# SamsungLabs/nb-asr

Measured on AMD Instinct MI355X. Metric: utterances_per_sec, higher is better.
Workload: dtype f32

## Files before the change

### nb_asr_amd/csrc/gemm_conv_split.hip

```cpp
#include "storage.h"

#include <cstdlib>

#include <type_traits>

namespace nbasr {

typedef float floatx4 __attribute__((ext_vector_type(4)));

constexpr int PB_CI = 16, PB_TAPS = 8;
constexpr int pb_frames(int nj) { return 64 * nj; }
constexpr int pb_rows(int mi) { return 32 * mi; }
constexpr int PB_THREADS = 512;

struct SplitBf16x3 {
    static constexpr int NS = 3;
    typedef __bf16 vec8 __attribute__((ext_vector_type(8)));
    static constexpr bool SCALED = false;
    __host__ __device__ static constexpr int taps_per_step(int stride) { return stride == 1 ? 4 : 2; }
    __device__ static __forceinline__ void split(float v, unsigned short (&s)[NS]) {
        const __bf16 hi = static_cast<__bf16>(v);
        const float r1 = v - static_cast<float>(hi);
        const __bf16 mid = static_cast<__bf16>(r1);
        const __bf16 lo = static_cast<__bf16>(r1 - static_cast<float>(mid));
        s[0] = __builtin_bit_cast(unsigned short, hi);
        s[1] = __builtin_bit_cast(unsigned short, mid);
        s[2] = __builtin_bit_cast(unsigned short, lo);
    }
    __device__ static __forceinline__ floatx4 mfma(vec8 a, vec8 b, floatx4 c) {
        return __builtin_amdgcn_mfma_f32_16x16x32_bf16(a, b, c, 0, 0, 0);
    }
    static constexpr const char* NAME = "nbasr_dense_conv1d_packed(bf16x3)";
};

struct SplitF16x2 {
    static constexpr int NS = 2;
    typedef _Float16 vec8 __attribute__((ext_vector_type(8)));
    static constexpr bool SCALED = true;
    __host__ __device__ static constexpr int taps_per_step(int) { return 4; }
    __device__ static __forceinline__ void split(float v, unsigned short (&s)[NS]) {
        const _Float16 hi = static_cast<_Float16>(v);
        const _Float16 lo = static_cast<_Float16>(v - static_cast<float>(hi));
        s[0] = __builtin_bit_cast(unsigned short, hi);
        s[1] = __builtin_bit_cast(unsigned short, lo);
    }
    __device__ static __forceinline__ floatx4 mfma(vec8 a, vec8 b, floatx4 c) {
        return __builtin_amdgcn_mfma_f32_16x16x32_f16(a, b, c, 0, 0, 0);
    }
    static constexpr const char* NAME = "nbasr_dense_conv1d_packed(f16x2)";
};

struct PlainBf16 {
    static constexpr int NS = 1;
    typedef __bf16 vec8 __attribute__((ext_vector_type(8)));
    static constexpr bool SCALED = false;
    __host__ __device__ static constexpr int taps_per_step(int) { return 8; }
    __device__ static __forceinline__ void split(float v, unsigned short (&s)[NS]) {
        s[0] = __builtin_bit_cast(unsigned short, static_cast<__bf16>(v));
    }
    __device__ static __forceinline__ floatx4 mfma(vec8 a, vec8 b, floatx4 c) {
        return __builtin_amdgcn_mfma_f32_16x16x32_bf16(a, b, c, 0, 0, 0);
    }
    static constexpr const char* NAME = "nbasr_dense_conv1d_packed(bf16)";
};

template <class P> constexpr bool has_image_path() { return P::SCALED || P::NS == 1; }

template <class P> constexpr size_t pb_group_bytes(int mi) { return static_cast<size_t>(P::NS) * PB_TAPS * pb_rows(mi) * PB_CI * 2; }

template <class P, int S, int MI = 4, int NJ = 4>
struct GeoP {
    static constexpr int PBM = pb_rows(MI);
    static constexpr int PBN = pb_frames(NJ);
    static constexpr int TP = P::taps_per_step(S);
    static constexpr int QSTEPS = PB_TAPS / TP;
    static constexpr int A_STEP_BYTES = P::NS * TP * PBM * PB_CI * 2;
    static constexpr int XR = (PBN - 1) * S + PB_TAPS;
    static constexpr int XRH = (XR + 1) / 2;
    static constexpr int ROWS = (S == 1) ? XR : 2 * XRH;
    static constexpr int RP = (ROWS + 15) / 16 * 16;
    static constexpr int X_BYTES = P::NS * RP * PB_CI * 2;
    static constexpr int NQUADS = ((XR + 3 + 3) / 4 + 7) / 8 * 8;
    static constexpr int XITEMS = NQUADS * (PB_CI / 2);
    static constexpr int NCHUNK = QSTEPS > 1 ? QSTEPS - 1 : 1;
    static constexpr int XI = (XITEMS + PB_THREADS * NCHUNK - 1) / (PB_THREADS * NCHUNK);
    static constexpr int RING = 2;
    static constexpr int OPERAND_BYTES = RING * (A_STEP_BYTES + X_BYTES);
    static constexpr int STAGING_BYTES = 8 * 32 * 68 * 4;
    static constexpr int LDS_BYTES = OPERAND_BYTES > STAGING_BYTES ? OPERAND_BYTES : STAGING_BYTES;
    __device__ static constexpr int rowmap(int row) { return (S == 1) ? row : (row & 1) * XRH + (row >> 1); }
};

struct PackedConvArgs {
    const float* x; const unsigned char* wp; const float* bias;
    const float* s0; const float* s1; const float* s2;
    float* y;
    int c_in, frames_in, ld_in, c_out, frames_out, ld_out, lpad;
    int n_groups, n_mt, n_nt, batch;
    LnRef ln_x;
    const float* x_absmax;
    const float* w_inv_scale;
    int x_is_image;
    const float* x_range;
    int sel_want;
    int staged_epilogue;
    float* part;
};

__device__ __forceinline__ bool range_is_extreme(const float* r) { return r[2] != 0.f || r[1] < r[0] * 2.44140625e-04f; }

__host__ __device__ inline void pow2_normaliser(float absmax, int target, float& scale, float& inv)
{
    unsigned bits;
    __builtin_memcpy(&bits, &absmax, 4);
    const int e = static_cast<int>((bits >> 23) & 0xffu);
    int k = (bits & 0x7fffffffu) ? (127 + target) - e : 0;
    k = k > 126 ? 126 : (k < -126 ? -126 : k);
    const unsigned sb = static_cast<unsigned>(127 + k) << 23, ib = static_cast<unsigned>(127 - k) << 23;
    __builtin_memcpy(&scale, &sb, 4);
    __builtin_memcpy(&inv, &ib, 4);
}

__device__ __forceinline__ unsigned pack2(unsigned short a, unsigned short b) {
    return static_cast<unsigned>(a) | (static_cast<unsigned>(b) << 16);
}

__global__ __launch_bounds__(256) void weight_row_scales_kernel(const float* __restrict__ w, float* __restrict__ scales,
                                                                int c_out, int row_elems, int rows)
{
    __shared__ float s_max[4];
    const int co = blockIdx.x;
    float m = 0.f;
    if (co < c_out)
        for (int i = threadIdx.x; i < row_elems; i += 256) m = fmaxf(m, fabsf(w[static_cast<size_t>(co) * row_elems + i]));
#pragma unroll
    for (int d = 32; d >= 1; d >>= 1) m = fmaxf(m, __shfl_xor(m, d));
    if ((threadIdx.x & 63) == 0) s_max[threadIdx.x >> 6] = m;
    __syncthreads();
    if (threadIdx.x == 0) {
        float scale, inv;
        pow2_normaliser(fmaxf(fmaxf(s_max[0], s_max[1]), fmaxf(s_max[2], s_max[3])), 13, scale, inv);
        scales[co] = scale;
        scales[rows + co] = inv;
    }
}

template <class P>
__global__ __launch_bounds__(256) void pack_dense_weights_kernel(const float* __restrict__ w, unsigned short* __restrict__ wp,
                                                                 const float* __restrict__ row_scale,
                                                                 int c_out, int c_in, int n_mt, int n_groups, int PB_TP, int PB_M)
{
    const int PB_QSTEPS = PB_TAPS / PB_TP;
    const long long total = static_cast<long long>(n_mt) * n_groups * PB_QSTEPS * PB_TP * PB_M * PB_CI;
    for (long long i = static_cast<long long>(blockIdx.x) * blockDim.x + threadIdx.x; i < total;
         i += static_cast<long long>(gridDim.x) * blockDim.x) {
        long long e = i;
        const int ci_l = e % PB_CI; e /= PB_CI;
        const int co_l = e % PB_M; e /= PB_M;
        const int tp = e % PB_TP; e /= PB_TP;
        const int q = e % PB_QSTEPS; e /= PB_QSTEPS;
        const int g = e % n_groups; e /= n_groups;
        const int mt = static_cast<int>(e);
        const int co = mt * PB_M + co_l, ci = g * PB_CI + ci_l, tap = q * PB_TP + tp;
        float v = (co < c_out && ci < c_in) ? w[(static_cast<size_t>(co) * c_in + ci) * PB_TAPS + tap] : 0.f;
        if (P::SCALED) v *= row_scale[co];
        unsigned short s[P::NS];
        P::split(v, s);
        const size_t step = (static_cast<size_t>(mt) * n_groups + g) * PB_QSTEPS + q;
#pragma unroll
        for (int k = 0; k < P::NS; ++k)
            wp[((((step * P::NS + k) * PB_TP + tp) * 2 + (ci_l >> 3)) * PB_M + co_l) * 8 + (ci_l & 7)] = s[k];
    }
}

template <class P, int S, bool LNX, bool XIMG = false, int MI = 4, int NJ = 4>
__global__ __launch_bounds__(PB_THREADS, 2) void gemm_conv_split_kernel(const PackedConvArgs a)
{
    static_assert(NJ == 4 || (NJ == 2 && XIMG && P::NS == 2) || (NJ == 8 && XIMG && P::NS == 1),
                  "128-frame tiles exist for the fp16 image path only, 512-frame tiles for the one-term bf16 flavour only");
    static_assert(!(XIMG && LNX) && !(XIMG && !has_image_path<P>()), "the image path: scaled fp16 scheme or plain bf16, no LayerNorm on load");
    static_assert(XIMG || P::NS > 1, "plain bf16 operands exist as an image only");
    static_assert(MI == 4 || ((MI == 5 || MI == 3 || MI == 2) && XIMG), "160-, 96- and 64-row tiles exist for the image path only");
    using G = GeoP<P, S, MI, NJ>;
    constexpr int PB_M = G::PBM, WROWS = 16 * MI;
    constexpr int PB_N = G::PBN, WCOLS = 16 * NJ;
    using vec8 = typename P::vec8;
    constexpr int TP = G::TP, QS = G::QSTEPS, ASTEP = G::A_STEP_BYTES;
    extern __shared__ __attribute__((aligned(16))) unsigned char smem[];
    unsigned char* const Abuf = smem;
    unsigned char* const Xbase = smem + G::RING * ASTEP;

    const int nwg = gridDim.x, id = blockIdx.x;
    const int xq = nwg >> 3, xr = nwg & 7, xcd = id & 7;
    const int L = (xcd < xr ? xcd * (xq + 1) : xr * (xq + 1) + (xcd - xr) * xq) + (id >> 3);
    int mt_i, b, nt_i;
    {
        mt_i = L % a.n_mt;
        const int rest = L / a.n_mt;
        b = rest / a.n_nt;
        nt_i = rest - b * a.n_nt;
    }
    const int m0 = mt_i * PB_M, n0 = nt_i * PB_N;
    if (a.x_range && a.sel_want >= 0 && static_cast<int>(range_is_extreme(a.x_range + 4 * b)) != a.sel_want) return;

    const int tid = threadIdx.x;
    const int lane = tid & 63;
    const int wave = __builtin_amdgcn_readfirstlane(tid >> 6);
    const int wm = wave >> 2, wn = wave & 3;
    const bool older = wave < 4;

    const float* __restrict__ xb = a.x + static_cast<size_t>(b) * a.c_in * a.ld_in;
    const int tin0 = n0 * S - a.lpad;
    const float* __restrict__ xstats = LNX ? a.ln_x.stats + static_cast<size_t>(b) * 2 * a.ld_in : nullptr;
    const unsigned char* __restrict__ wtile = a.wp + static_cast<size_t>(mt_i) * a.n_groups * pb_group_bytes<P>(MI);

    const bool wave_active = (m0 + wm * WROWS) < a.c_out && (n0 + wn * WCOLS) < a.ld_out;

    floatx4 acc[MI][NJ], tot[MI][NJ];
#pragma unroll
    for (int i = 0; i < MI; ++i)
#pragma unroll
        for (int j = 0; j < NJ; ++j)
#pragma unroll
            for (int r = 0; r < 4; ++r) { acc[i][j][r] = 0.f; tot[i][j][r] = 0.f; }
    auto flush_group = [&]() {
        if constexpr (P::NS > 1) {
#pragma unroll
            for (int i = 0; i < MI; ++i)
#pragma unroll
                for (int j = 0; j < NJ; ++j)
#pragma unroll
                    for (int r = 0; r < 4; ++r) { tot[i][j][r] += acc[i][j][r]; acc[i][j][r] = 0.f; }
        }
    };

    auto dma_weights = [&](int step, int buf) {
        const unsigned char* src = wtile + static_cast<size_t>(step) * ASTEP;
#pragma unroll
        for (int j = 0; j < ASTEP / 1024 / 8; ++j) {
            const int chunk = wave * (ASTEP / 1024 / 8) + j;
            __builtin_amdgcn_global_load_lds(
                (const __attribute__((address_space(1))) void*)(src + chunk * 1024 + lane * 16),
                (__attribute__((address_space(3))) void*)(Abuf + buf * ASTEP + chunk * 1024),
                16, 0, 0);
        }
    };
    auto dma_x = [&](int g, int xbuf, int q) {
        constexpr int NP = (G::X_BYTES + 1023) / 1024;
        const unsigned char* img = reinterpret_cast<const unsigned char*>(a.x) +
                                   (static_cast<size_t>(b) * a.n_groups + g) * (2 * P::NS) * static_cast<size_t>(a.ld_in + 1) * 16;
#pragma unroll 1
        for (int i = wave * QS + q; i < NP; i += 8 * QS) {
            const int o = i * 1024 + lane * 16;
            if (o < G::X_BYTES) {
                const int plane = o / (G::RP * 16), rr = (o - plane * (G::RP * 16)) >> 4;
                const int frame = tin0 + (S == 1 ? rr : 2 * (rr % G::XRH) + rr / G::XRH);
                const int row = (rr < G::ROWS && frame >= 0 && frame < a.ld_in) ? frame + 1 : 0;
                __builtin_amdgcn_global_load_lds(
                    (const __attribute__((address_space(1))) void*)(img + (static_cast<size_t>(plane) * (a.ld_in + 1) + row) * 16),
                    (__attribute__((address_space(3))) void*)(Xbase + xbuf * G::X_BYTES + i * 1024), 16, 0, 0);
            }
        }
    };
    floatx4 xreg[G::XI][2];
    const int a0 = tin0 & ~3, xoff = tin0 - a0;
    float x_scale = 1.f, x_inv = 1.f;
    if constexpr (P::SCALED) pow2_normaliser(a.x_range ? a.x_range[4 * b] : a.x_absmax[b], 14, x_scale, x_inv);
    auto load_x = [&](int g, int c) {
#pragma unroll
        for (int i = 0; i < G::XI; ++i) {
            const int e = tid + PB_THREADS * (c * G::XI + i);
            const int p = (e >> 3) & 7;
            const int t = a0 + 4 * ((e >> 6) * 8 + (e & 7));
            const int ci = g * PB_CI + 2 * p;
            const bool ok = e < G::XITEMS && t >= 0 && t < a.ld_in;
            floatx4 v0 = {0.f, 0.f, 0.f, 0.f}, v1 = {0.f, 0.f, 0.f, 0.f};
            if (ok && ci < a.c_in) v0 = *reinterpret_cast<const floatx4*>(xb + static_cast<size_t>(ci) * a.ld_in + t);
            if (ok && ci + 1 < a.c_in) v1 = *reinterpret_cast<const floatx4*>(xb + static_cast<size_t>(ci + 1) * a.ld_in + t);
            if (LNX && ok) {
                const floatx4 mean = *reinterpret_cast<const floatx4*>(xstats + t);
                const floatx4 rstd = *reinterpret_cast<const floatx4*>(xstats + a.ld_in + t);
                if (ci < a.c_in) {
                    const float gm = a.ln_x.gamma[ci], bt = a.ln_x.beta[ci];
#pragma unroll
                    for (int j = 0; j < 4; ++j) v0[j] = ln_apply(v0[j], mean[j], rstd[j], gm, bt);
                }
                if (ci + 1 < a.c_in) {
                    const float gm = a.ln_x.gamma[ci + 1], bt = a.ln_x.beta[ci + 1];
#pragma unroll
                    for (int j = 0; j < 4; ++j) v1[j] = ln_apply(v1[j], mean[j], rstd[j], gm, bt);
                }
            }
            if constexpr (P::SCALED) { v0 *= x_scale; v1 *= x_scale; }
            xreg[i][0] = v0;
            xreg[i][1] = v1;
        }
    };
    auto commit_x = [&](int xbuf, int c) {
        unsigned* const X = reinterpret_cast<unsigned*>(Xbase + xbuf * G::X_BYTES);
#pragma unroll
        for (int i = 0; i < G::XI; ++i) {
            const int e = tid + PB_THREADS * (c * G::XI + i);
            const int p = (e >> 3) & 7;
            const int row0 = 4 * ((e >> 6) * 8 + (e & 7)) - xoff;
            if (e >= G::XITEMS) continue;
            unsigned* const col = X + (p >> 2) * G::RP * 4 + (p & 3);
#pragma unroll
            for (int j = 0; j < 4; ++j) {
                const int row = row0 + j;
                if (row < 0 || row >= G::XR) continue;
                unsigned short s0[P::NS], s1[P::NS];
                P::split(xreg[i][0][j], s0);
                P::split(xreg[i][1][j], s1);
                unsigned* dst = col + G::rowmap(row) * 4;
#pragma unroll
                for (int k = 0; k < P::NS; ++k) dst[k * 2 * G::RP * 4] = pack2(s0[k], s1[k]);
            }
        }
    };

    const int l15 = lane & 15, kq = lane >> 4;
    const int a_lane = (((kq >> 1) * 2 + (kq & 1)) * PB_M + wm * WROWS + l15) * 16;
    const int x_lane = (kq & 1) * G::RP * 16;

    constexpr bool PIPE = P::NS <= 2;
    auto mma_step = [&](int q, int abuf, int xbuf) {
        const unsigned char* A = Abuf + abuf * ASTEP + a_lane;
        const unsigned char* X = Xbase + xbuf * G::X_BYTES + x_lane;
        auto read_b = [&](int pp, int j, vec8 (&f)[P::NS]) {
            const int row = G::rowmap((wn * WCOLS + j * 16 + l15) * S + q * TP + 2 * pp + (kq >> 1));
#pragma unroll
            for (int k = 0; k < P::NS; ++k) f[k] = *reinterpret_cast<const vec8*>(X + (k * 2 * G::RP + row) * 16);
        };
        auto read_a = [&](int pp, int i, vec8 (&f)[P::NS]) {
#pragma unroll
            for (int k = 0; k < P::NS; ++k) f[k] = *reinterpret_cast<const vec8*>(A + ((k * TP + 2 * pp) * 2 * PB_M + i * 16) * 16);
        };
        auto block = [&](int i, int j, const vec8 (&af)[P::NS], const vec8 (&bf)[P::NS]) {
            floatx4 c = acc[i][j];
            if constexpr (P::NS == 3) {
                c = P::mfma(af[2], bf[0], c);
                c = P::mfma(af[0], bf[2], c);
                c = P::mfma(af[1], bf[1], c);
            }
            if constexpr (P::NS > 1) {
                c = P::mfma(af[1], bf[0], c);
                c = P::mfma(af[0], bf[1], c);
            }
            acc[i][j] = P::mfma(af[0], bf[0], c);
        };
        if constexpr (PIPE) {
            vec8 bfr[NJ][P::NS], af[2][P::NS];
#pragma unroll
            for (int j = 0; j < NJ; ++j) read_b(0, j, bfr[j]);
            read_a(0, 0, af[0]);
#pragma unroll
            for (int pp = 0; pp < TP / 2; ++pp) {
#pragma unroll
                for (int i = 0; i < MI; ++i) {
                    const int cur = (pp * MI + i) & 1;
                    const bool more_a = i < MI - 1 || pp + 1 < TP / 2;
#pragma unroll
                    for (int j = 0; j < NJ; ++j) {
                        __builtin_amdgcn_sched_barrier(0);
                        block(i, j, af[cur], bfr[j]);
                        __builtin_amdgcn_sched_barrier(0);
                        if (j == 0 && more_a) read_a(i < MI - 1 ? pp : pp + 1, (i + 1) % MI, af[cur ^ 1]);
                        if (i == MI - 1 && pp + 1 < TP / 2) read_b(pp + 1, j, bfr[j]);
                    }
                }
            }
            __builtin_amdgcn_sched_barrier(0);
        } else {
#pragma unroll 1
            for (int pp = 0; pp < TP / 2; ++pp) {
                vec8 bfr[NJ][P::NS];
#pragma unroll
                for (int j = 0; j < NJ; ++j) read_b(pp, j, bfr[j]);
#pragma unroll
                for (int i = 0; i < MI; ++i) {
                    vec8 af[P::NS];
                    read_a(pp, i, af);
#pragma unroll
                    for (int j = 0; j < NJ; ++j) block(i, j, af, bfr[j]);
                }
            }
        }
    };

    const int ng = a.n_groups;
    dma_weights(0, 0);
    if constexpr (XIMG) {
#pragma unroll 1
        for (int q = 0; q < QS; ++q) dma_x(0, 0, q);
    } else {
#pragma unroll 1
        for (int c = 0; c < G::NCHUNK; ++c) { load_x(0, c); commit_x(0, c); }
    }
    asm volatile("s_waitcnt vmcnt(0)" ::: "memory");
    __syncthreads();

    if (!older) __builtin_amdgcn_s_setprio(1);
    int step = 0;
    for (int g = 0; g < ng; ++g) {
        const bool more = g + 1 < ng;
#pragma unroll 1
        for (int q = 0; q < QS; ++q, ++step) {
            const bool prefetch = q + 1 < QS || more;
            const bool chunk = more && q < QS - 1;
            if (older) {
                if constexpr (XIMG) {
                    if (more) dma_x(g + 1, (g + 1) & 1, q);
                } else {
                    if (more && q >= 1) commit_x((g + 1) & 1, q - 1);
                    if (chunk) load_x(g + 1, q);
                }
                if (prefetch) dma_weights(step + 1, (step + 1) & 1);
            } else if (!XIMG && chunk) {
                load_x(g + 1, q);
            }
            if (wave_active) mma_step(q, step & 1, g & 1);
            if (!older) {
                if constexpr (XIMG) {
                    if (more) dma_x(g + 1, (g + 1) & 1, q);
                } else {
                    if (chunk) commit_x((g + 1) & 1, q);
                }
                if (prefetch) dma_weights(step + 1, (step + 1) & 1);
            }
            asm volatile("s_waitcnt vmcnt(0)" ::: "memory");
            __syncthreads();
        }
        flush_group();
    }

    if constexpr (P::NS == 1) {
        constexpr int TSH = WCOLS + 8;
        constexpr int LPR = WCOLS / 8, RPI = 64 / LPR;
        unsigned short* const T = reinterpret_cast<unsigned short*>(smem) + wave * (32 * TSH);
        static_assert(8 * 32 * TSH * 2 <= G::LDS_BYTES, "output staging must fit the operand buffers");
        if (wave_active) {
            bf16_t* const yb = reinterpret_cast<bf16_t*>(a.y);
            const int n = n0 + wn * WCOLS + (lane % LPR) * 8;
#pragma unroll
            for (int i0 = 0; i0 < MI; i0 += 2) {
#pragma unroll
                for (int ii = 0; ii < 2; ++ii) {
                    const int i = i0 + ii;
                    if (i >= MI) break;
#pragma unroll
                    for (int j = 0; j < NJ; ++j) {
                        const bool live = n0 + wn * WCOLS + j * 16 + l15 < a.frames_out;
#pragma unroll
                        for (int r = 0; r < 4; ++r) {
                            const int m = m0 + wm * WROWS + i * 16 + kq * 4 + r;
                            const float v = (live && m < a.c_out) ? relu_clamp(acc[i][j][r] + a.bias[m]) : 0.f;
                            T[(ii * 16 + kq * 4 + r) * TSH + j * 16 + l15] = __builtin_bit_cast(unsigned short, static_cast<__bf16>(v));
                        }
                    }
                }
                asm volatile("s_waitcnt lgkmcnt(0)" ::: "memory");
                const int rows_pass = (MI - i0 >= 2) ? 32 : 16;
#pragma unroll
                for (int it = 0; it < 32 / RPI; ++it) {
                    const int ml = it * RPI + lane / LPR, m = m0 + wm * WROWS + i0 * 16 + ml;
                    if (ml < rows_pass && m < a.c_out && n < a.ld_out) {
                        const u4v t = *reinterpret_cast<const u4v*>(T + ml * TSH + (lane % LPR) * 8);
                        *reinterpret_cast<u4v*>(yb + (static_cast<size_t>(b) * a.c_out + m) * a.ld_out + n) = t;
                    }
                }
                asm volatile("s_waitcnt lgkmcnt(0)" ::: "memory");
            }
        }
        return;
    } else {
    if (!a.s0 && !a.s1 && !a.s2 && a.staged_epilogue) {
        constexpr int TS = WCOLS + 4;
        constexpr int FQ = WCOLS / 4, RI = 64 / FQ, NIT = 32 / RI;
        float* const T = reinterpret_cast<float*>(smem) + wave * (32 * TS);
        static_assert(8 * 32 * TS * 4 <= G::LDS_BYTES, "output staging must fit the operand buffers");
        if (!wave_active) return;
        const int nc = n0 + wn * WCOLS + (lane % FQ) * 4;
        const bool want_stats = a.part != nullptr;
        const int scol = lane % WCOLS, usel = lane / WCOLS;
        const int ncol = n0 + wn * WCOLS + scol;
#pragma unroll
        for (int i0 = 0; i0 < MI; i0 += 2) {
#pragma unroll
            for (int ii = 0; ii < 2; ++ii) {
                const int i = i0 + ii;
                if (i >= MI) break;
#pragma unroll
                for (int j = 0; j < NJ; ++j) {
                    const bool live = n0 + wn * WCOLS + j * 16 + l15 < a.frames_out;
#pragma unroll
                    for (int r = 0; r < 4; ++r) {
                        const int m = m0 + wm * WROWS + i * 16 + kq * 4 + r;
                        float v = 0.f;
                        if (live && m < a.c_out) {
                            float sum = tot[i][j][r];
                            if constexpr (P::SCALED) sum = sum * x_inv * a.w_inv_scale[m];
                            v = relu_clamp(sum + a.bias[m]);
                        }
                        T[(ii * 16 + kq * 4 + r) * TS + j * 16 + l15] = v;
                    }
                }
            }
            asm volatile("s_waitcnt lgkmcnt(0)" ::: "memory");
            const int rows_pass = (MI - i0 >= 2) ? 32 : 16;
#pragma unroll
            for (int it = 0; it < NIT; ++it) {
                const int ml = it * RI + lane / FQ;
                const int m = m0 + wm * WROWS + i0 * 16 + ml;
                if (ml < rows_pass && m < a.c_out && nc < a.ld_out) {
                    const floatx4 t = *reinterpret_cast<const floatx4*>(T + ml * TS + (lane % FQ) * 4);
                    *reinterpret_cast<floatx4*>(a.y + (static_cast<size_t>(b) * a.c_out + m) * a.ld_out + nc) = t;
                }
            }
            if (want_stats) {
#pragma unroll
                for (int u0 = 0; u0 < 2; u0 += 64 / WCOLS) {
                    const int u = u0 + usel;
                    const int mu = m0 + wm * WROWS + (i0 + u) * 16;
                    if (i0 + u < MI && mu < a.c_out) {
                        const int nrows = min(16, a.c_out - mu);
                        const float c = T[(u * 16) * TS + scol];
                        float s1 = 0.f, s2 = 0.f;
#pragma unroll
                        for (int r = 1; r < 16; ++r) {
                            const float d = (r < nrows) ? T[(u * 16 + r) * TS + scol] - c : 0.f;
                            s1 += d;
                            s2 = __builtin_fmaf(d, d, s2);
                        }
                        if (ncol < a.ld_out) {
                            const float inv = 1.0f / static_cast<float>(nrows);
                            float* prow = a.part + (static_cast<size_t>(mu >> 4) * a.batch + b) * 2 * a.ld_out + ncol;
                            prow[0] = c + s1 * inv;
                            prow[a.ld_out] = s2 - s1 * s1 * inv;
                        }
                    }
                }
            }
            asm volatile("s_waitcnt lgkmcnt(0)" ::: "memory");
        }
        return;
    }
    if (!wave_active) return;
#pragma unroll
    for (int i = 0; i < MI; ++i) {
#pragma unroll
        for (int j = 0; j < NJ; ++j) {
            const int n = n0 + wn * WCOLS + j * 16 + l15;
            if (n >= a.ld_out) continue;
            const bool live = n < a.frames_out;
#pragma unroll
            for (int r = 0; r < 4; ++r) {
                const int m = m0 + wm * WROWS + i * 16 + kq * 4 + r;
                if (m >= a.c_out) continue;
                float sum = tot[i][j][r];
                if constexpr (P::SCALED) sum = sum * x_inv * a.w_inv_scale[m];
                float v = relu_clamp(sum + a.bias[m]);
                const size_t off = (static_cast<size_t>(b) * a.c_out + m) * a.ld_out + n;
                if (a.s0) v += a.s0[off];
                if (a.s1) v += a.s1[off];
                if (a.s2) v += a.s2[off];
                a.y[off] = live ? v : 0.f;
            }
        }
    }
    }
}


template <class P, int S>
static int launch_packed(PackedConvArgs a, hipStream_t stream)
{
    using G = GeoP<P, S>;
    constexpr int PB_M = G::PBM;
    constexpr bool HAS_LNX = !P::SCALED;
    static const hipError_t attr0 = hipFuncSetAttribute(reinterpret_cast<const void*>(gemm_conv_split_kernel<P, S, false>),
                                                        hipFuncAttributeMaxDynamicSharedMemorySize, G::LDS_BYTES);
    static const hipError_t attr1 = hipFuncSetAttribute(reinterpret_cast<const void*>(gemm_conv_split_kernel<P, S, HAS_LNX>),
                                                        hipFuncAttributeMaxDynamicSharedMemorySize, G::LDS_BYTES);
    const hipError_t attr = attr0 != hipSuccess ? attr0 : attr1;
    if (attr != hipSuccess) {
        set_error("%s: cannot reserve %d bytes of LDS: %s", P::NAME, G::LDS_BYTES, hipGetErrorString(attr));
        return static_cast<int>(attr);
    }
    NBASR_REQUIRE(HAS_LNX || !a.ln_x.stats, NBASR_EINVAL, "%s: this scheme takes no deferred LayerNorm", P::NAME);
    a.n_mt = (a.c_out + PB_M - 1) / PB_M;
    a.n_nt = (a.ld_out + G::PBN - 1) / G::PBN;
    const long long nwg = static_cast<long long>(a.n_mt) * a.n_nt * a.batch;
    NBASR_REQUIRE(nwg < (1ll << 31), NBASR_EINVAL, "%s: too many tiles (%lld)", P::NAME, nwg);
    if (a.ln_x.stats)
        hipLaunchKernelGGL((gemm_conv_split_kernel<P, S, HAS_LNX>), dim3(static_cast<unsigned>(nwg)), dim3(PB_THREADS), G::LDS_BYTES, stream, a);
    else
        hipLaunchKernelGGL((gemm_conv_split_kernel<P, S, false>), dim3(static_cast<unsigned>(nwg)), dim3(PB_THREADS), G::LDS_BYTES, stream, a);
    return launch_status(P::NAME);
}

static inline int rows_to_mi(int row_tile) { return row_tile == 128 ? 4 : (row_tile == 160 ? 5 : (row_tile == 96 ? 3 : (row_tile == 64 ? 2 : 0))); }

template <class P, int S, int MI, int NJ = 4>
static int launch_image(PackedConvArgs a, hipStream_t stream)
{
    using G = GeoP<P, S, MI, NJ>;
    static const hipError_t attr = hipFuncSetAttribute(reinterpret_cast<const void*>(gemm_conv_split_kernel<P, S, false, true, MI, NJ>),
                                                       hipFuncAttributeMaxDynamicSharedMemorySize, G::LDS_BYTES);
    if (attr != hipSuccess) {
        set_error("%s: cannot reserve %d bytes of LDS: %s", P::NAME, G::LDS_BYTES, hipGetErrorString(attr));
        return static_cast<int>(attr);
    }
    a.n_mt = (a.c_out + G::PBM - 1) / G::PBM;
    a.n_nt = (a.ld_out + G::PBN - 1) / G::PBN;
    const long long nwg = static_cast<long long>(a.n_mt) * a.n_nt * a.batch;
    NBASR_REQUIRE(nwg < (1ll << 31), NBASR_EINVAL, "%s: too many tiles (%lld)", P::NAME, nwg);
    hipLaunchKernelGGL((gemm_conv_split_kernel<P, S, false, true, MI, NJ>), dim3(static_cast<unsigned>(nwg)), dim3(PB_THREADS), G::LDS_BYTES, stream, a);
    return launch_status(P::NAME);
}

template <class P>
static size_t packed_bytes(int c_out, int c_in, int kernel, int row_tile = 128)
{
    const int mi = rows_to_mi(row_tile);
    if (c_out <= 0 || c_in <= 0 || kernel != PB_TAPS || mi == 0 || (mi != 4 && !has_image_path<P>())) return 0;
    const size_t PB_M = pb_rows(mi), n_mt = (c_out + PB_M - 1) / PB_M, n_groups = (c_in + PB_CI - 1) / PB_CI;
    return n_mt * n_groups * pb_group_bytes<P>(mi) + (P::SCALED ? 2 * n_mt * PB_M * sizeof(float) : 0);
}

template <class P>
static int pack_impl(const float* w, void* packed, int c_out, int c_in, int kernel, int stride, nbasr_stream_t stream, int row_tile = 128)
{
    clear_error();
    const int mi = rows_to_mi(row_tile);
    NBASR_REQUIRE(mi != 0 && (mi == 4 || has_image_path<P>()), NBASR_EINVAL, "nbasr_pack_dense_weights: row_tile=%d unsupported (128, or 64 / 96 / 160 for the image-path schemes)", row_tile);
    const int PB_M = pb_rows(mi);
    NBASR_REQUIRE(c_out > 0 && c_in > 0, NBASR_EINVAL, "nbasr_pack_dense_weights: bad sizes");
    NBASR_REQUIRE(kernel == PB_TAPS && (stride == 1 || stride == 2), NBASR_EINVAL,
                  "nbasr_pack_dense_weights: (kernel=%d, stride=%d) unsupported (the downsample convs have k=8, s in {1,2})", kernel, stride);
    NBASR_REQUIRE(w && packed, NBASR_ENULL, "nbasr_pack_dense_weights: NULL pointer");
    NBASR_REQUIRE(aligned16(packed), NBASR_EALIGN, "nbasr_pack_dense_weights: packed buffer must be 16-byte aligned");
    const int n_mt = (c_out + PB_M - 1) / PB_M, n_groups = (c_in + PB_CI - 1) / PB_CI;
    float* scales = nullptr;
    if (P::SCALED) {
        scales = reinterpret_cast<float*>(static_cast<unsigned char*>(packed) + static_cast<size_t>(n_mt) * n_groups * pb_group_bytes<P>(mi));
        hipLaunchKernelGGL(weight_row_scales_kernel, dim3(n_mt * PB_M), dim3(256), 0, as_stream(stream), w, scales, c_out,
                           c_in * PB_TAPS, n_mt * PB_M);
    }
    hipLaunchKernelGGL(pack_dense_weights_kernel<P>, dim3(2048), dim3(256), 0, as_stream(stream), w,
                       static_cast<unsigned short*>(packed), scales, c_out, c_in, n_mt, n_groups, P::taps_per_step(stride), PB_M);
    return launch_status("nbasr_pack_dense_weights");
}

template <class P>
static int dense_packed_impl(const float* x, const void* packed_w, const float* bias, const float* skip0,
                             const float* skip1, const float* skip2, float* y, int batch, int c_in,
                             int frames_in, int ld_in, int c_out, int ld_out, int kernel, int stride,
                             const nbasr_deferred_ln* ln, const float* x_absmax, nbasr_stream_t stream, bool x_is_image = false,
                             int row_tile = 128, const float* x_range = nullptr, int sel_want = -1, float* stats_part = nullptr,
                             int frame_tile = 256)
{
    clear_error();
    const int mi = rows_to_mi(row_tile);
    NBASR_REQUIRE(mi == 4 || ((mi == 5 || mi == 3 || mi == 2) && x_is_image && P::SCALED), NBASR_EINVAL,
                  "%s: row_tile=%d unsupported (128; 64, 96 and 160 for the fp16 image path)", P::NAME, row_tile);
    const int PB_M = pb_rows(mi);
    NBASR_REQUIRE(frame_tile == 256 || (frame_tile == 128 && x_is_image && P::SCALED), NBASR_EINVAL,
                  "%s: frame_tile=%d unsupported (256; 128 for the fp16 image path)", P::NAME, frame_tile);
    NBASR_REQUIRE(batch >= 0 && c_in > 0 && c_out > 0 && frames_in >= 0, NBASR_EINVAL, "%s: bad sizes", P::NAME);
    NBASR_REQUIRE(kernel == PB_TAPS && (stride == 1 || stride == 2), NBASR_EINVAL,
                  "%s: (kernel=%d, stride=%d) unsupported; packed path covers k=8, s in {1,2}", P::NAME, kernel, stride);
    const int frames_out = (frames_in + stride - 1) / stride;
    NBASR_REQUIRE(ld_in >= frames_in, NBASR_EINVAL, "%s: ld_in=%d < frames_in=%d", P::NAME, ld_in, frames_in);
    NBASR_REQUIRE(ld_in % 4 == 0, NBASR_EALIGN, "%s: ld_in=%d must be a multiple of 4", P::NAME, ld_in);
    NBASR_REQUIRE(ld_out >= frames_out && ld_out % 4 == 0, NBASR_EALIGN,
                  "%s: ld_out=%d must be >= %d output frames and a multiple of 4", P::NAME, ld_out, frames_out);
    if (batch == 0 || frames_out == 0) return NBASR_OK;
    NBASR_REQUIRE(x && packed_w && bias && y, NBASR_ENULL, "%s: x, packed_w, bias, y must be non-NULL", P::NAME);
    NBASR_REQUIRE(aligned16(packed_w) && aligned16(x), NBASR_EALIGN, "%s: x and packed weights must be 16-byte aligned", P::NAME);
    PackedConvArgs a{};
    a.x = x; a.wp = static_cast<const unsigned char*>(packed_w); a.bias = bias; a.s0 = skip0; a.s1 = skip1; a.s2 = skip2; a.y = y;
    a.c_in = c_in; a.frames_in = frames_in; a.ld_in = ld_in; a.c_out = c_out; a.frames_out = frames_out; a.ld_out = ld_out;
    a.lpad = pad_left(kernel, 1, stride); a.n_groups = (c_in + PB_CI - 1) / PB_CI; a.batch = batch;
    NBASR_REQUIRE(!ln || (ln->stats && ln->gamma && ln->beta), NBASR_ENULL, "%s: deferred LayerNorm needs stats, gamma and beta", P::NAME);
    a.ln_x = ln_ref(ln, true);
    a.x_range = x_range;
    a.sel_want = x_range ? sel_want : -1;
    a.staged_epilogue = 1;
    NBASR_REQUIRE(!stats_part || (!skip0 && !skip1 && !skip2 && aligned16(stats_part)), NBASR_EINVAL,
                  "%s: the statistics by-product exists for the skip-free convolution only (stats_part 16-byte aligned)", P::NAME);
    a.part = stats_part;
    if (P::SCALED) {
        NBASR_REQUIRE(x_absmax || x_range, NBASR_ENULL, "%s: x_absmax (per-utterance bound of |x|) must be non-NULL", P::NAME);
        a.x_absmax = x_absmax;
        a.x_is_image = x_is_image ? 1 : 0;
        a.w_inv_scale = reinterpret_cast<const float*>(a.wp + static_cast<size_t>((c_out + PB_M - 1) / PB_M) * a.n_groups * pb_group_bytes<P>(mi))
                        + static_cast<size_t>((c_out + PB_M - 1) / PB_M) * PB_M;
    }
    if constexpr (has_image_path<P>() && P::SCALED) {
        if (x_is_image) {
            hipStream_t s = as_stream(stream);
            if (frame_tile == 128) {
                switch (mi) {
                    case 5: return stride == 1 ? launch_image<P, 1, 5, 2>(a, s) : launch_image<P, 2, 5, 2>(a, s);
                    case 3: return stride == 1 ? launch_image<P, 1, 3, 2>(a, s) : launch_image<P, 2, 3, 2>(a, s);
                    case 2: return stride == 1 ? launch_image<P, 1, 2, 2>(a, s) : launch_image<P, 2, 2, 2>(a, s);
                    default: return stride == 1 ? launch_image<P, 1, 4, 2>(a, s) : launch_image<P, 2, 4, 2>(a, s);
                }
            }
            switch (mi) {
                case 5: return stride == 1 ? launch_image<P, 1, 5>(a, s) : launch_image<P, 2, 5>(a, s);
                case 3: return stride == 1 ? launch_image<P, 1, 3>(a, s) : launch_image<P, 2, 3>(a, s);
                case 2: return stride == 1 ? launch_image<P, 1, 2>(a, s) : launch_image<P, 2, 2>(a, s);
                default: return stride == 1 ? launch_image<P, 1, 4>(a, s) : launch_image<P, 2, 4>(a, s);
            }
        }
    }
    return stride == 1 ? launch_packed<P, 1>(a, as_stream(stream)) : launch_packed<P, 2>(a, as_stream(stream));
}

}

using namespace nbasr;

extern "C" size_t nbasr_split_image_bytes(int batch, int channels, int ld)
{
    if (batch <= 0 || channels <= 0 || ld < 0) return 0;
    return static_cast<size_t>(batch) * ((channels + PB_CI - 1) / PB_CI) * 4 * (static_cast<size_t>(ld) + 1) * 16;
}

extern "C" size_t nbasr_packed_dense_weights_bytes(int scheme, int c_out, int c_in, int kernel, int row_tile)
{
    switch (scheme) {
        case NBASR_DENSE_BF16X3: return packed_bytes<SplitBf16x3>(c_out, c_in, kernel, row_tile);
        case NBASR_DENSE_F16X2:  return packed_bytes<SplitF16x2>(c_out, c_in, kernel, row_tile);
        case NBASR_DENSE_BF16:   return packed_bytes<PlainBf16>(c_out, c_in, kernel, row_tile);
        default: return 0;
    }
}

extern "C" int nbasr_pack_dense_weights(int scheme, const float* w, void* packed, int c_out, int c_in, int kernel, int stride, int row_tile,
                                        nbasr_stream_t stream)
{
    switch (scheme) {
        case NBASR_DENSE_BF16X3: return pack_impl<SplitBf16x3>(w, packed, c_out, c_in, kernel, stride, stream, row_tile);
        case NBASR_DENSE_F16X2:  return pack_impl<SplitF16x2>(w, packed, c_out, c_in, kernel, stride, stream, row_tile);
        case NBASR_DENSE_BF16:   return pack_impl<PlainBf16>(w, packed, c_out, c_in, kernel, stride, stream, row_tile);
        default: break;
    }
    clear_error();
    NBASR_REQUIRE(false, NBASR_EINVAL, "nbasr_pack_dense_weights: unknown scheme %d", scheme);
    return NBASR_EINVAL;
}

static int dense_bf16_image_impl(const void* x_image, const void* packed_w, const float* bias, void* y, int batch, int c_in,
                                 int frames_in, int ld_in, int c_out, int ld_out, int kernel, int stride, int row_tile, int frame_tile,
                                 nbasr_stream_t stream)
{
    using P = PlainBf16;
    clear_error();
    const int mi = rows_to_mi(row_tile);
    NBASR_REQUIRE(mi == 4 || mi == 5, NBASR_EINVAL, "%s: row_tile=%d unsupported (128 or 160)", P::NAME, row_tile);
    NBASR_REQUIRE(batch >= 0 && c_in > 0 && c_out > 0 && frames_in >= 0, NBASR_EINVAL, "%s: bad sizes", P::NAME);
    NBASR_REQUIRE(kernel == PB_TAPS && (stride == 1 || stride == 2), NBASR_EINVAL,
                  "%s: (kernel=%d, stride=%d) unsupported; the downsample convs have k=8, s in {1,2}", P::NAME, kernel, stride);
    const int frames_out = (frames_in + stride - 1) / stride;
    NBASR_REQUIRE(ld_in >= frames_in, NBASR_EINVAL, "%s: ld_in=%d < frames_in=%d", P::NAME, ld_in, frames_in);
    NBASR_REQUIRE(ld_out >= frames_out && ld_out % 8 == 0, NBASR_EALIGN,
                  "%s: ld_out=%d must be >= %d output frames and a multiple of 8", P::NAME, ld_out, frames_out);
    if (batch == 0 || frames_out == 0) return NBASR_OK;
    NBASR_REQUIRE(x_image && packed_w && bias && y, NBASR_ENULL, "%s: x_image, packed_w, bias, y must be non-NULL", P::NAME);
    NBASR_REQUIRE(aligned16(packed_w) && aligned16(x_image) && aligned16(y), NBASR_EALIGN, "%s: pointers must be 16-byte aligned", P::NAME);
    PackedConvArgs a{};
    a.x = static_cast<const float*>(x_image); a.wp = static_cast<const unsigned char*>(packed_w); a.bias = bias;
    a.y = static_cast<float*>(y);
    a.c_in = c_in; a.frames_in = frames_in; a.ld_in = ld_in; a.c_out = c_out; a.frames_out = frames_out; a.ld_out = ld_out;
    a.lpad = pad_left(kernel, 1, stride); a.n_groups = (c_in + PB_CI - 1) / PB_CI; a.batch = batch;
    a.ln_x = LnRef{nullptr, nullptr, nullptr};
    a.x_is_image = 1;
    hipStream_t s = as_stream(stream);
    if (frame_tile == 512) {
        if (mi == 5) return stride == 1 ? launch_image<P, 1, 5, 8>(a, s) : launch_image<P, 2, 5, 8>(a, s);
        return stride == 1 ? launch_image<P, 1, 4, 8>(a, s) : launch_image<P, 2, 4, 8>(a, s);
    }
    if (mi == 5) return stride == 1 ? launch_image<P, 1, 5>(a, s) : launch_image<P, 2, 5>(a, s);
    return stride == 1 ? launch_image<P, 1, 4>(a, s) : launch_image<P, 2, 4>(a, s);
}

extern "C" int nbasr_dense_conv1d_packed(int scheme, const void* x, int x_is_image, const float* x_absmax, const float* x_range,
                                         const void* packed_w, const float* bias, const float* skip0, const float* skip1,
                                         const float* skip2, void* y, int batch, int c_in, int frames_in, int ld_in, int c_out,
                                         int ld_out, int kernel, int stride, int row_tile, int frame_tile, const nbasr_deferred_ln* ln,
                                         float* stats_part, nbasr_stream_t stream)
{
    clear_error();
    const float* xf = static_cast<const float*>(x);
    float* yf = static_cast<float*>(y);
    const bool image = x_is_image != 0;
    switch (scheme) {
        case NBASR_DENSE_BF16X3:
            NBASR_REQUIRE(!image && !x_absmax, NBASR_EINVAL, "nbasr_dense_conv1d_packed: the bf16x3 scheme reads a plain fp32 tensor and takes no bound");
            return dense_packed_impl<SplitBf16x3>(xf, packed_w, bias, skip0, skip1, skip2, yf, batch, c_in, frames_in, ld_in, c_out, ld_out,
                                                  kernel, stride, ln, nullptr, stream, false, row_tile, x_range, 1, stats_part, frame_tile);
        case NBASR_DENSE_F16X2:
            NBASR_REQUIRE(!ln, NBASR_EINVAL, "nbasr_dense_conv1d_packed: the fp16x2 scheme takes no pending LayerNorm (nbasr_layernorm_split_image writes its operand)");
            NBASR_REQUIRE(!(image && (skip0 || skip1 || skip2)), NBASR_EINVAL, "nbasr_dense_conv1d_packed: the image path takes no skips");
            NBASR_REQUIRE(!(x_absmax && x_range), NBASR_EINVAL, "nbasr_dense_conv1d_packed: give x_absmax or x_range, not both");
            return dense_packed_impl<SplitF16x2>(xf, packed_w, bias, skip0, skip1, skip2, yf, batch, c_in, frames_in, ld_in, c_out, ld_out,
                                                 kernel, stride, nullptr, x_absmax, stream, image, row_tile, x_range, 0, stats_part, frame_tile);
        case NBASR_DENSE_BF16:
            NBASR_REQUIRE(frame_tile == 256 || frame_tile == 512, NBASR_EINVAL, "nbasr_dense_conv1d_packed: the bf16 scheme has 256- and 512-frame tiles");
            NBASR_REQUIRE(image && !x_absmax && !x_range && !ln && !skip0 && !skip1 && !skip2 && !stats_part, NBASR_EINVAL,
                          "nbasr_dense_conv1d_packed: the bf16 scheme reads nbasr_bf16_image's operand image only (no bound, range, LayerNorm, skips or statistics)");
            return dense_bf16_image_impl(x, packed_w, bias, y, batch, c_in, frames_in, ld_in, c_out, ld_out, kernel, stride, row_tile, frame_tile, stream);
        default: break;
    }
    NBASR_REQUIRE(false, NBASR_EINVAL, "nbasr_dense_conv1d_packed: unknown scheme %d", scheme);
    return NBASR_EINVAL;
}
```

### nb_asr_amd/csrc/gemm_pointwise.hip

```cpp
#include "storage.h"

namespace nbasr {

typedef float floatx4 __attribute__((ext_vector_type(4)));
typedef _Float16 pw_h2 __attribute__((ext_vector_type(2)));

constexpr int PW_M = 128, PW_N = 256, PW_K = 32;
constexpr int PW_THREADS = 512;

__device__ __forceinline__ float pw_load(const float* p) { return *p; }
__device__ __forceinline__ float pw_load(const bf16_t* p) { return __uint_as_float(static_cast<unsigned>(p->bits) << 16); }
__device__ __forceinline__ void pw_store(float* p, float v) { *p = v; }
__device__ __forceinline__ void pw_store(bf16_t* p, float v) { p->bits = static_cast<unsigned short>(pack_bf16x2(v, 0.f) & 0xffffu); }

template <int TERMS>
struct PwSteps {
    static constexpr int NS = TERMS;
    static constexpr int A_STEP = TERMS * 2 * 2 * PW_M * 16;
    static constexpr int X_STEP = TERMS * 2 * 2 * PW_N * 16;
    static constexpr int RING = 3;
    static constexpr int LDS = RING * (A_STEP + X_STEP);
    static constexpr int DMA_PER_WAVE = 3 * TERMS;
};

struct PwF16x2 : PwSteps<2> {
    typedef _Float16 vec8 __attribute__((ext_vector_type(8)));
    typedef float act_t;
    static constexpr bool SCALED = true;
    static constexpr bool ORDER_BY_HOST = true;
    static constexpr int LD_ALIGN = 4, PROJECTION_LD_ALIGN = 1;
    __device__ static __forceinline__ void split2(float a, float b, unsigned (&d)[NS]) {
        const _Float16 ha = static_cast<_Float16>(a), hb = static_cast<_Float16>(b);
        d[0] = __builtin_bit_cast(unsigned, pw_h2{ha, hb});
        d[1] = __builtin_bit_cast(unsigned, pw_h2{static_cast<_Float16>((a - static_cast<float>(ha)) * 2048.f),
                                                  static_cast<_Float16>((b - static_cast<float>(hb)) * 2048.f)});
    }
    __device__ static __forceinline__ floatx4 mfma(vec8 a, vec8 b, floatx4 c) { return __builtin_amdgcn_mfma_f32_16x16x32_f16(a, b, c, 0, 0, 0); }
};

struct PwBf16 : PwSteps<1> {
    typedef __bf16 vec8 __attribute__((ext_vector_type(8)));
    typedef bf16_t act_t;
    static constexpr bool SCALED = false;
    static constexpr bool ORDER_BY_HOST = false;
    static constexpr int LD_ALIGN = 8, PROJECTION_LD_ALIGN = 8;
    __device__ static __forceinline__ void split2(float a, float b, unsigned (&d)[NS]) { d[0] = pack_bf16x2(a, b); }
    __device__ static __forceinline__ floatx4 mfma(vec8 a, vec8 b, floatx4 c) { return __builtin_amdgcn_mfma_f32_16x16x32_bf16(a, b, c, 0, 0, 0); }
};

__host__ __device__ inline void pw_pow2(float absmax, int target, float& scale, float& inv)
{
    unsigned bits;
    __builtin_memcpy(&bits, &absmax, 4);
    const int e = static_cast<int>((bits >> 23) & 0xffu);
    int k = (bits & 0x7fffffffu) ? (127 + target) - e : 0;
    k = k > 126 ? 126 : (k < -126 ? -126 : k);
    const unsigned sb = static_cast<unsigned>(127 + k) << 23, ib = static_cast<unsigned>(127 - k) << 23;
    __builtin_memcpy(&scale, &sb, 4);
    __builtin_memcpy(&inv, &ib, 4);
}

__global__ __launch_bounds__(256) void pw_row_scales_kernel(const float* __restrict__ w, float* __restrict__ scales, int c_out,
                                                            int c_in, int rows)
{
    __shared__ float s_max[4];
    const int co = blockIdx.x;
    float m = 0.f;
    if (co < c_out)
        for (int i = threadIdx.x; i < c_in; i += 256) m = fmaxf(m, fabsf(w[static_cast<size_t>(co) * c_in + i]));
#pragma unroll
    for (int d = 32; d >= 1; d >>= 1) m = fmaxf(m, __shfl_xor(m, d));
    if ((threadIdx.x & 63) == 0) s_max[threadIdx.x >> 6] = m;
    __syncthreads();
    if (threadIdx.x == 0) {
        float scale, inv;
        pw_pow2(fmaxf(fmaxf(s_max[0], s_max[1]), fmaxf(s_max[2], s_max[3])), 13, scale, inv);
        scales[co] = scale;
        scales[rows + co] = inv;
    }
}

template <class P>
__global__ __launch_bounds__(256) void pw_pack_weights_kernel(const float* __restrict__ w, unsigned short* __restrict__ wp,
                                                              const float* __restrict__ row_scale, int c_out, int c_in,
                                                              int n_mt, int n_ks)
{
    const long long total = static_cast<long long>(n_mt) * n_ks * PW_M * PW_K;
    for (long long i = static_cast<long long>(blockIdx.x) * blockDim.x + threadIdx.x; i < total;
         i += static_cast<long long>(gridDim.x) * blockDim.x) {
        long long e = i;
        const int ci_l = e % PW_K; e /= PW_K;
        const int co_l = e % PW_M; e /= PW_M;
        const int ks = e % n_ks; e /= n_ks;
        const int mt = static_cast<int>(e);
        const int co = mt * PW_M + co_l, ci = ks * PW_K + ci_l;
        float v = 0.f;
        if (co < c_out && ci < c_in) v = P::SCALED ? w[static_cast<size_t>(co) * c_in + ci] * row_scale[co] : w[static_cast<size_t>(co) * c_in + ci];
        unsigned d[P::NS];
        P::split2(v, 0.f, d);
        const int blk = ci_l >> 4, half = (ci_l >> 3) & 1, c8 = ci_l & 7;
        const size_t step = static_cast<size_t>(mt) * n_ks + ks;
        const size_t base = step * (P::A_STEP / 2) + ((static_cast<size_t>(blk) * 2 + half) * PW_M + co_l) * 8 + c8;
#pragma unroll
        for (int s = 0; s < P::NS; ++s) wp[base + s * (P::A_STEP / 2 / P::NS)] = static_cast<unsigned short>(d[s] & 0xffffu);
    }
}


template <bool LNX, class T>
__device__ __forceinline__ void pw_fetch32(const T* __restrict__ x, int c_in, int frames, int ld, const LnRef& ln, float (&v)[PW_K])
{
    const int ci0 = blockIdx.y * PW_K, b = blockIdx.z;
    const int t = blockIdx.x * PW_N + threadIdx.x;
    const bool live = t < frames;
    const T* __restrict__ xb = x + static_cast<size_t>(b) * c_in * ld + t;
    float mean = 0.f, rstd = 0.f;
    if (LNX && live) {
        const float* st = ln.stats + static_cast<size_t>(b) * 2 * ld;
        mean = st[t]; rstd = st[ld + t];
    }
#pragma unroll
    for (int c = 0; c < PW_K; ++c) {
        const int ci = ci0 + c;
        v[c] = (live && ci < c_in) ? pw_load(xb + static_cast<size_t>(ci) * ld) : 0.f;
    }
    if (LNX) {
#pragma unroll
        for (int c = 0; c < PW_K; ++c) {
            const int ci = ci0 + c;
            if (live && ci < c_in) v[c] = ln_apply(v[c], mean, rstd, ln.gamma[ci], ln.beta[ci]);
        }
    }
}

template <bool LNX>
__global__ __launch_bounds__(256) void pw_tile_max_kernel(const float* __restrict__ x, float* __restrict__ partial, int c_in,
                                                          int frames, int ld, int n_ks, const LnRef ln)
{
    __shared__ float s_max[4];
    float v[PW_K];
    pw_fetch32<LNX>(x, c_in, frames, ld, ln, v);
    float m = 0.f;
#pragma unroll
    for (int c = 0; c < PW_K; ++c) m = fmaxf(m, fabsf(v[c]));
#pragma unroll
    for (int d = 32; d >= 1; d >>= 1) m = fmaxf(m, __shfl_xor(m, d));
    if ((threadIdx.x & 63) == 0) s_max[threadIdx.x >> 6] = m;
    __syncthreads();
    if (threadIdx.x == 0)
        partial[(static_cast<size_t>(blockIdx.z) * gridDim.x + blockIdx.x) * n_ks + blockIdx.y] = fmaxf(fmaxf(s_max[0], s_max[1]), fmaxf(s_max[2], s_max[3]));
}

template <class P, bool LNX>
__global__ __launch_bounds__(256) void pw_presplit_kernel(const typename P::act_t* __restrict__ x, unsigned char* __restrict__ image,
                                                          float* __restrict__ inv_scale, const float* __restrict__ partial,
                                                          int c_in, int frames, int ld, int n_ks, const LnRef ln)
{
    const int nt = blockIdx.x, ks = blockIdx.y, b = blockIdx.z;
    const int lane_t = threadIdx.x;
    float v[PW_K];
    pw_fetch32<LNX>(x, c_in, frames, ld, ln, v);
    float scale = 1.f;
    if constexpr (P::SCALED) {
        const float* __restrict__ pt = partial + (static_cast<size_t>(b) * gridDim.x + nt) * n_ks;
        float tile_max = 0.f;
        for (int i = threadIdx.x & 63; i < n_ks; i += 64) tile_max = fmaxf(tile_max, pt[i]);
#pragma unroll
        for (int d = 32; d >= 1; d >>= 1) tile_max = fmaxf(tile_max, __shfl_xor(tile_max, d));
        float inv;
        pw_pow2(tile_max, 14, scale, inv);
        if (threadIdx.x == 0 && ks == 0) inv_scale[static_cast<size_t>(b) * gridDim.x + nt] = inv;
    }
    unsigned char* step = image + ((static_cast<size_t>(b) * gridDim.x + nt) * n_ks + ks) * P::X_STEP;
#pragma unroll
    for (int bh = 0; bh < 4; ++bh) {
        u4v term[P::NS];
#pragma unroll
        for (int q = 0; q < 4; ++q) {
            const float v0 = v[bh * 8 + 2 * q], v1 = v[bh * 8 + 2 * q + 1];
            unsigned d[P::NS];
            if constexpr (P::SCALED) P::split2(v0 * scale, v1 * scale, d);
            else P::split2(v0, v1, d);
#pragma unroll
            for (int s = 0; s < P::NS; ++s) term[s][q] = d[s];
        }
        unsigned char* row = step + (bh * PW_N + lane_t) * 16;
#pragma unroll
        for (int s = 0; s < P::NS; ++s) *reinterpret_cast<u4v*>(row + s * (P::X_STEP / P::NS)) = term[s];
    }
}

template <class P>
struct PointwiseArgs {
    const unsigned char* image; const float* x_inv; const unsigned char* wp; const float* w_inv;
    const float* bias; const float* bias2;
    const typename P::act_t* s0; const typename P::act_t* s1; const typename P::act_t* s2;
    void* y;
    int c_out, frames, ld_out, n_ks, n_mt, n_nt, batch;
    int n_major;
    int row_stride_t, row_stride_b;
    LnRef ln_s0;
};

template <class P, bool SWAP, bool RELU>
__global__ __launch_bounds__(PW_THREADS, 2) void pw_gemm_kernel(const PointwiseArgs<P> a)
{
    typedef typename P::vec8 vec8;
    typedef typename P::act_t act_t;
    constexpr int NS = P::NS, A_STEP = P::A_STEP, X_STEP = P::X_STEP;
    extern __shared__ __attribute__((aligned(16))) unsigned char smem[];
    unsigned char* const Abuf = smem;
    unsigned char* const Xbuf = smem + P::RING * A_STEP;

    const int nwg = gridDim.x, id = blockIdx.x;
    const int xq = nwg >> 3, xr = nwg & 7, xcd = id & 7;
    const int L = (xcd < xr ? xcd * (xq + 1) : xr * (xq + 1) + (xcd - xr) * xq) + (id >> 3);
    int mt_i, b, nt_i;
    if (!P::ORDER_BY_HOST || a.n_major) {
        const int ntg = L / a.n_mt;
        mt_i = L - ntg * a.n_mt;
        b = ntg / a.n_nt;
        nt_i = ntg - b * a.n_nt;
    } else {
        const int per_m = a.n_nt * a.batch;
        mt_i = L / per_m;
        const int rem = L - mt_i * per_m;
        b = rem / a.n_nt;
        nt_i = rem - b * a.n_nt;
    }
    const int m0 = mt_i * PW_M, n0 = nt_i * PW_N;

    const int tid = threadIdx.x, lane = tid & 63;
    const int wave = __builtin_amdgcn_readfirstlane(tid >> 6);
    const int wm = wave >> 2, wn = wave & 3;
    const int l15 = lane & 15, kq = lane >> 4;
    const bool wave_active = (m0 + wm * 64) < a.c_out && (n0 + wn * 64) < a.ld_out;

    const unsigned char* __restrict__ wsrc = a.wp + static_cast<size_t>(mt_i) * a.n_ks * A_STEP;
    const unsigned char* __restrict__ xsrc = a.image + (static_cast<size_t>(b) * a.n_nt + nt_i) * a.n_ks * X_STEP;

    floatx4 big[4][4], small[4][4];
#pragma unroll
    for (int i = 0; i < 4; ++i)
#pragma unroll
        for (int j = 0; j < 4; ++j)
#pragma unroll
            for (int r = 0; r < 4; ++r) { big[i][j][r] = 0.f; small[i][j][r] = 0.f; }

    auto dma_step = [&](int ks, int buf) {
        const unsigned char* ws = wsrc + static_cast<size_t>(ks) * A_STEP;
        const unsigned char* xs = xsrc + static_cast<size_t>(ks) * X_STEP;
#pragma unroll
        for (int j = 0; j < NS; ++j) {
            const int piece = wave * NS + j;
            __builtin_amdgcn_global_load_lds((const __attribute__((address_space(1))) void*)(ws + piece * 1024 + lane * 16),
                                             (__attribute__((address_space(3))) void*)(Abuf + buf * A_STEP + piece * 1024), 16, 0, 0);
        }
#pragma unroll
        for (int j = 0; j < 2 * NS; ++j) {
            const int piece = wave * 2 * NS + j;
            __builtin_amdgcn_global_load_lds((const __attribute__((address_space(1))) void*)(xs + piece * 1024 + lane * 16),
                                             (__attribute__((address_space(3))) void*)(Xbuf + buf * X_STEP + piece * 1024), 16, 0, 0);
        }
    };

    const int a_lane = ((kq * PW_M) + wm * 64 + l15) * 16;
    const int x_lane = ((kq * PW_N) + wn * 64 + l15) * 16;

    auto mma_step = [&](int buf) {
        const unsigned char* A = Abuf + buf * A_STEP + a_lane;
        const unsigned char* X = Xbuf + buf * X_STEP + x_lane;
        auto read_a = [&](int i, vec8 (&f)[NS]) {
#pragma unroll
            for (int s = 0; s < NS; ++s) f[s] = *reinterpret_cast<const vec8*>(A + s * (A_STEP / NS) + i * 16 * 16);
        };
        vec8 bt[4][NS], at[2][NS];
#pragma unroll
        for (int j = 0; j < 4; ++j)
#pragma unroll
            for (int s = 0; s < NS; ++s) bt[j][s] = *reinterpret_cast<const vec8*>(X + s * (X_STEP / NS) + j * 16 * 16);
        read_a(0, at[0]);
#pragma unroll
        for (int i = 0; i < 4; ++i) {
#pragma unroll
            for (int j = 0; j < 4; ++j) {
                __builtin_amdgcn_sched_barrier(0);
                if constexpr (NS == 2) {
                    floatx4 c = small[i][j];
                    c = P::mfma(at[i & 1][1], bt[j][0], c);
                    c = P::mfma(at[i & 1][0], bt[j][1], c);
                    small[i][j] = c;
                }
                big[i][j] = P::mfma(at[i & 1][0], bt[j][0], big[i][j]);
                __builtin_amdgcn_sched_barrier(0);
                if (j == 0 && i < 3) read_a(i + 1, at[(i + 1) & 1]);
            }
        }
        __builtin_amdgcn_sched_barrier(0);
    };

    const bool older = wave < 4;
    const int n_ks = a.n_ks;
    dma_step(0, 0);
    if (n_ks > 1) {
        dma_step(1, 1);
        asm volatile("s_waitcnt vmcnt(%0)\n\ts_barrier" :: "n"(P::DMA_PER_WAVE) : "memory");
    } else {
        asm volatile("s_waitcnt vmcnt(0)\n\ts_barrier" ::: "memory");
    }
    if (!older) __builtin_amdgcn_s_setprio(1);
    int buf = 0;
#pragma unroll 1
    for (int ks = 0; ks < n_ks; ++ks) {
        const bool ahead = ks + 2 < n_ks;
        const int fill = buf == 0 ? 2 : buf - 1;
        if (older && ahead) dma_step(ks + 2, fill);
        if (wave_active) mma_step(buf);
        if (!older && ahead) dma_step(ks + 2, fill);
        if (ahead) asm volatile("s_waitcnt vmcnt(%0) lgkmcnt(0)\n\ts_barrier" :: "n"(P::DMA_PER_WAVE) : "memory");
        else       asm volatile("s_waitcnt vmcnt(0) lgkmcnt(0)\n\ts_barrier" ::: "memory");
        buf = buf == 2 ? 0 : buf + 1;
    }
    if (!older) __builtin_amdgcn_s_setprio(0);

    if (!wave_active) return;
    float x_inv = 1.f;
    if constexpr (P::SCALED) x_inv = a.x_inv[static_cast<size_t>(b) * a.n_nt + nt_i];
    auto product = [&](int i, int j, int r, int m) {
        float v = big[i][j][r];
        if constexpr (NS == 2) v += small[i][j][r] * (1.f / 2048.f);
        if constexpr (P::SCALED) v = v * x_inv * a.w_inv[m];
        return v;
    };
    if constexpr (SWAP) {
        constexpr int TS = 64 + 4;
        static_assert(8 * 16 * TS * 4 <= P::LDS, "output staging must fit the operand buffers");
        float* const T = reinterpret_cast<float*>(smem) + wave * (16 * TS);
        const int mseg = m0 + wm * 64 + l15 * 4;
#pragma unroll
        for (int j = 0; j < 4; ++j) {
#pragma unroll
            for (int i = 0; i < 4; ++i) {
                const int mb = m0 + wm * 64 + i * 16 + kq * 4;
                floatx4 o;
#pragma unroll
                for (int r = 0; r < 4; ++r) {
                    const int m = mb + r;
                    float v = 0.f;
                    if (m < a.c_out) {
                        v = product(i, j, r, m) + a.bias[m];
                        if (a.bias2) v += a.bias2[m];
                        if (RELU) v = relu_clamp(v);
                    }
                    o[r] = v;
                }
                *reinterpret_cast<floatx4*>(T + l15 * TS + i * 16 + kq * 4) = o;
            }
            asm volatile("s_waitcnt lgkmcnt(0)" ::: "memory");
#pragma unroll
            for (int it = 0; it < 4; ++it) {
                const int row = it * 4 + kq;
                const int n = n0 + wn * 64 + j * 16 + row;
                if (n >= a.frames || mseg >= a.c_out) continue;
                const floatx4 o = *reinterpret_cast<const floatx4*>(T + row * TS + l15 * 4);
                float* dst = static_cast<float*>(a.y) + (static_cast<size_t>(n) * a.row_stride_t + static_cast<size_t>(b) * a.row_stride_b) * a.c_out + mseg;
                *reinterpret_cast<floatx4*>(dst) = o;
            }
            asm volatile("s_waitcnt lgkmcnt(0)" ::: "memory");
        }
        return;
    }
#pragma unroll
    for (int i = 0; i < 4; ++i) {
#pragma unroll
        for (int j = 0; j < 4; ++j) {
            const int n = n0 + wn * 64 + j * 16 + l15;
            const int mb = m0 + wm * 64 + i * 16 + kq * 4;
            if (n >= a.ld_out) continue;
            const bool live = n < a.frames;
            float s0m = 0.f, s0r = 0.f;
            if (a.s0 && a.ln_s0.stats) {
                const float* st = a.ln_s0.stats + static_cast<size_t>(b) * 2 * a.ld_out;
                s0m = st[n]; s0r = st[a.ld_out + n];
            }
            act_t* yb = static_cast<act_t*>(a.y);
#pragma unroll
            for (int r = 0; r < 4; ++r) {
                const int m = mb + r;
                if (m >= a.c_out) continue;
                float v = product(i, j, r, m) + a.bias[m];
                if (RELU) v = relu_clamp(v);
                const size_t off = (static_cast<size_t>(b) * a.c_out + m) * a.ld_out + n;
                if (a.s0) v += a.ln_s0.stats ? ln_apply(pw_load(a.s0 + off), s0m, s0r, a.ln_s0.gamma[m], a.ln_s0.beta[m]) : pw_load(a.s0 + off);
                if (a.s1) v += pw_load(a.s1 + off);
                if (a.s2) v += pw_load(a.s2 + off);
                pw_store(yb + off, live ? v : 0.f);
            }
        }
    }
}

static inline int pw_n_ks(int c_in) { return (c_in + PW_K - 1) / PW_K; }
static inline int pw_n_mt(int c_out) { return (c_out + PW_M - 1) / PW_M; }
static inline int pw_n_nt(int ld) { return (ld + PW_N - 1) / PW_N; }
static inline size_t pw_round4(size_t n) { return (n + 3) & ~static_cast<size_t>(3); }
template <class P> static size_t pw_image_bytes(int batch, int c_in, int ld) { return static_cast<size_t>(batch) * pw_n_nt(ld) * pw_n_ks(c_in) * P::X_STEP; }
template <class P> static size_t pw_weight_image_bytes(int c_out, int c_in) { return static_cast<size_t>(pw_n_mt(c_out)) * pw_n_ks(c_in) * P::A_STEP; }

template <class P>
static size_t pw_weights_bytes(int c_out, int c_in)
{
    if (c_out <= 0 || c_in <= 0) return 0;
    return pw_weight_image_bytes<P>(c_out, c_in) + (P::SCALED ? 2 * static_cast<size_t>(pw_n_mt(c_out)) * PW_M * sizeof(float) : 0);
}

template <class P>
static size_t pw_workspace_bytes(int batch, int c_in, int ld)
{
    if (batch <= 0 || c_in <= 0 || ld <= 0) return 0;
    const size_t tiles = static_cast<size_t>(batch) * pw_n_nt(ld);
    return pw_image_bytes<P>(batch, c_in, ld) + (P::SCALED ? (pw_round4(tiles) + tiles * pw_n_ks(c_in)) * sizeof(float) : 0);
}

template <class P>
static int pw_pack(const char* what, const float* w, void* packed, int c_out, int c_in, nbasr_stream_t stream)
{
    clear_error();
    NBASR_REQUIRE(c_out > 0 && c_in > 0, NBASR_EINVAL, "%s: bad sizes", what);
    NBASR_REQUIRE(w && packed, NBASR_ENULL, "%s: NULL pointer", what);
    NBASR_REQUIRE(aligned16(packed), NBASR_EALIGN, "%s: packed buffer must be 16-byte aligned", what);
    const int n_mt = pw_n_mt(c_out), n_ks = pw_n_ks(c_in);
    float* scales = nullptr;
    if (P::SCALED) {
        scales = reinterpret_cast<float*>(static_cast<unsigned char*>(packed) + pw_weight_image_bytes<P>(c_out, c_in));
        hipLaunchKernelGGL(pw_row_scales_kernel, dim3(n_mt * PW_M), dim3(256), 0, as_stream(stream), w, scales, c_out, c_in, n_mt * PW_M);
    }
    hipLaunchKernelGGL(pw_pack_weights_kernel<P>, dim3(1024), dim3(256), 0, as_stream(stream), w, static_cast<unsigned short*>(packed), scales,
                       c_out, c_in, n_mt, n_ks);
    return launch_status(what);
}

template <class P, bool LNX>
static int pw_image(const typename P::act_t* x, void* ws, int batch, int c_in, int frames, int ld, LnRef ln, hipStream_t stream, const char* what)
{
    unsigned char* image = static_cast<unsigned char*>(ws);
    float* inv = nullptr;
    float* partial = nullptr;
    const int n_ks = pw_n_ks(c_in);
    const dim3 grid(pw_n_nt(ld), n_ks, batch);
    if constexpr (P::SCALED) {
        inv = reinterpret_cast<float*>(image + pw_image_bytes<P>(batch, c_in, ld));
        partial = inv + pw_round4(static_cast<size_t>(batch) * pw_n_nt(ld));
        hipLaunchKernelGGL(pw_tile_max_kernel<LNX>, grid, dim3(256), 0, stream, x, partial, c_in, frames, ld, n_ks, ln);
    }
    hipLaunchKernelGGL((pw_presplit_kernel<P, LNX>), grid, dim3(256), 0, stream, x, image, inv, partial, c_in, frames, ld, n_ks, ln);
    return launch_status(what);
}

static int pw_checks(const char* what, const void* x, const void* ws, const void* packed_w, const float* bias, const void* y,
                     int batch, int c_in, int frames, int ld, int c_out)
{
    NBASR_REQUIRE(batch >= 0 && c_in > 0 && c_out > 0 && frames >= 0 && ld >= frames, NBASR_EINVAL, "%s: bad sizes", what);
    if (batch == 0 || frames == 0) return 1;
    NBASR_REQUIRE(batch <= 65535, NBASR_EINVAL, "%s: batch %d > 65535", what, batch);
    NBASR_REQUIRE(x && ws && packed_w && bias && y, NBASR_ENULL, "%s: x, workspace, packed_w, bias, y must be non-NULL", what);
    NBASR_REQUIRE(aligned16(ws) && aligned16(packed_w), NBASR_EALIGN, "%s: workspace and packed weights must be 16-byte aligned", what);
    return NBASR_OK;
}

template <class P, bool SWAP, bool RELU>
static int pw_run(const char* what, const typename P::act_t* x, void* ws, const void* packed_w, PointwiseArgs<P> a, int batch, int c_in,
                  int frames, int ld, int c_out, LnRef ln_x, hipStream_t stream)
{
    const int rc = ln_x.stats ? pw_image<P, true>(x, ws, batch, c_in, frames, ld, ln_x, stream, what)
                              : pw_image<P, false>(x, ws, batch, c_in, frames, ld, ln_x, stream, what);
    if (rc != NBASR_OK) return rc;
    a.image = static_cast<const unsigned char*>(ws);
    a.wp = static_cast<const unsigned char*>(packed_w);
    a.n_mt = pw_n_mt(c_out); a.n_ks = pw_n_ks(c_in); a.n_nt = pw_n_nt(ld);
    if (P::SCALED) {
        a.x_inv = reinterpret_cast<const float*>(a.image + pw_image_bytes<P>(batch, c_in, ld));
        a.w_inv = reinterpret_cast<const float*>(a.wp + pw_weight_image_bytes<P>(c_out, c_in)) + static_cast<size_t>(a.n_mt) * PW_M;
    }
    a.c_out = c_out; a.frames = frames; a.ld_out = ld; a.batch = batch;

    static const hipError_t attr = hipFuncSetAttribute(reinterpret_cast<const void*>(pw_gemm_kernel<P, SWAP, RELU>),
                                                       hipFuncAttributeMaxDynamicSharedMemorySize, P::LDS);
    if (attr != hipSuccess) {
        set_error("%s: cannot reserve %d bytes of LDS: %s", what, P::LDS, hipGetErrorString(attr));
        return static_cast<int>(attr);
    }
    const long long nwg = static_cast<long long>(a.n_mt) * a.n_nt * a.batch;
    NBASR_REQUIRE(nwg < (1ll << 31), NBASR_EINVAL, "%s: too many tiles (%lld)", what, nwg);
    a.n_major = static_cast<long long>(a.n_mt) * P::A_STEP <= static_cast<long long>(a.n_nt) * a.batch * P::X_STEP ? 1 : 0;
    hipLaunchKernelGGL((pw_gemm_kernel<P, SWAP, RELU>), dim3(static_cast<unsigned>(nwg)), dim3(PW_THREADS), P::LDS, stream, a);
    return launch_status(what);
}

template <class P>
static int pw_linear(const char* what, const typename P::act_t* x, void* ws, const void* packed_w, const float* bias,
                     const typename P::act_t* skip0, const typename P::act_t* skip1, const typename P::act_t* skip2, typename P::act_t* y,
                     int batch, int c_in, int frames, int ld, int c_out, const nbasr_deferred_ln* ln, int ln_on_x, int ln_on_skip0,
                     nbasr_stream_t stream)
{
    clear_error();
    const int rc0 = pw_checks(what, x, ws, packed_w, bias, y, batch, c_in, frames, ld, c_out);
    if (rc0 != NBASR_OK) return rc0 == 1 ? NBASR_OK : rc0;
    NBASR_REQUIRE(ld % P::LD_ALIGN == 0, NBASR_EALIGN, "%s: ld=%d must be a multiple of %d (rows are pitched to 16 bytes)", what, ld, P::LD_ALIGN);
    const bool any_ln = ln && (ln_on_x || (ln_on_skip0 && skip0));
    NBASR_REQUIRE(!any_ln || (ln->stats && ln->gamma && ln->beta), NBASR_ENULL, "%s: deferred LayerNorm needs stats, gamma and beta", what);
    NBASR_REQUIRE(!(ln && ln_on_x && ln_on_skip0 && skip0) || c_in == c_out, NBASR_EINVAL, "%s: one descriptor for x and skip0 needs equal shapes", what);
    PointwiseArgs<P> a{};
    a.bias = bias; a.s0 = skip0; a.s1 = skip1; a.s2 = skip2; a.y = y;
    a.ln_s0 = ln_ref(ln, ln_on_skip0 != 0 && skip0 != nullptr);
    return pw_run<P, false, true>(what, x, ws, packed_w, a, batch, c_in, frames, ld, c_out, ln_ref(ln, ln_on_x != 0), as_stream(stream));
}

template <class P>
static int pw_projection(const char* what, const typename P::act_t* x, void* ws, const void* packed_w_ih, const float* b_ih, const float* b_hh,
                         float* gates_ws, int batch, int c_in, int frames, int ld, int hidden, const nbasr_deferred_ln* ln, int batch_total,
                         int batch_offset, nbasr_stream_t stream)
{
    const int rc0 = pw_checks(what, x, ws, packed_w_ih, b_ih, gates_ws, batch, c_in, frames, ld, 4 * hidden);
    if (rc0 != NBASR_OK) return rc0 == 1 ? NBASR_OK : rc0;
    NBASR_REQUIRE(b_hh != nullptr, NBASR_ENULL, "%s: b_hh is NULL", what);
    NBASR_REQUIRE(hidden % 4 == 0 && aligned16(gates_ws) && ld % P::PROJECTION_LD_ALIGN == 0, NBASR_EALIGN,
                  "%s: hidden %% 4, ld %% %d and 16-byte aligned gates_ws required", what, P::PROJECTION_LD_ALIGN);
    NBASR_REQUIRE(!ln || (ln->stats && ln->gamma && ln->beta), NBASR_ENULL, "%s: deferred LayerNorm needs stats, gamma and beta", what);
    PointwiseArgs<P> a{};
    a.bias = b_ih; a.bias2 = b_hh; a.y = gates_ws + static_cast<size_t>(batch_offset) * 4 * hidden;
    a.row_stride_t = batch_total; a.row_stride_b = 1;
    return pw_run<P, true, false>(what, x, ws, packed_w_ih, a, batch, c_in, frames, ld, 4 * hidden, ln_ref(ln, true), as_stream(stream));
}

}

using namespace nbasr;

extern "C" size_t nbasr_pointwise_packed_weights_bytes(int c_out, int c_in) { return pw_weights_bytes<PwF16x2>(c_out, c_in); }
extern "C" size_t nbasr_pointwise_bf16_weights_bytes(int c_out, int c_in) { return pw_weights_bytes<PwBf16>(c_out, c_in); }
extern "C" size_t nbasr_pointwise_workspace_bytes(int batch, int c_in, int ld) { return pw_workspace_bytes<PwF16x2>(batch, c_in, ld); }
extern "C" size_t nbasr_pointwise_bf16_workspace_bytes(int batch, int c_in, int ld) { return pw_workspace_bytes<PwBf16>(batch, c_in, ld); }

extern "C" int nbasr_pack_pointwise_weights(const float* w, void* packed, int c_out, int c_in, nbasr_stream_t stream)
{
    return pw_pack<PwF16x2>("nbasr_pack_pointwise_weights", w, packed, c_out, c_in, stream);
}

extern "C" int nbasr_pack_pointwise_weights_bf16(const float* w, void* packed, int c_out, int c_in, nbasr_stream_t stream)
{
    return pw_pack<PwBf16>("nbasr_pack_pointwise_weights_bf16", w, packed, c_out, c_in, stream);
}

extern "C" int nbasr_linear_fused_packed(const float* x, void* ws, const void* packed_w, const float* bias, const float* skip0,
                                         const float* skip1, const float* skip2, float* y, int batch, int channels_in,
                                         int frames, int ld, int channels_out, const nbasr_deferred_ln* ln, int ln_on_x,
                                         int ln_on_skip0, nbasr_stream_t stream)
{
    return pw_linear<PwF16x2>("nbasr_linear_fused_packed", x, ws, packed_w, bias, skip0, skip1, skip2, y, batch, channels_in, frames, ld,
                              channels_out, ln, ln_on_x, ln_on_skip0, stream);
}

extern "C" int nbasr_linear_fused_bf16(const void* x, void* ws, const void* packed_w, const float* bias, const void* skip0,
                                       const void* skip1, const void* skip2, void* y, int batch, int channels_in, int frames, int ld,
                                       int channels_out, const nbasr_deferred_ln* ln, int ln_on_x, int ln_on_skip0, nbasr_stream_t stream)
{
    return pw_linear<PwBf16>("nbasr_linear_fused_bf16", static_cast<const bf16_t*>(x), ws, packed_w, bias, static_cast<const bf16_t*>(skip0),
                             static_cast<const bf16_t*>(skip1), static_cast<const bf16_t*>(skip2), static_cast<bf16_t*>(y), batch, channels_in,
                             frames, ld, channels_out, ln, ln_on_x, ln_on_skip0, stream);
}

extern "C" int nbasr_lstm_input_projection_packed(const float* x, void* ws, const void* packed_w_ih, const float* b_ih,
                                                  const float* b_hh, float* gates_ws, int batch, int c_in, int frames, int ld,
                                                  int hidden, const nbasr_deferred_ln* ln, nbasr_stream_t stream)
{
    clear_error();
    return pw_projection<PwF16x2>("nbasr_lstm_input_projection_packed", x, ws, packed_w_ih, b_ih, b_hh, gates_ws, batch, c_in, frames, ld, hidden,
                                  ln, batch, 0, stream);
}

extern "C" int nbasr_lstm_input_projection_packed_into(const float* x, void* ws, const void* packed_w_ih, const float* b_ih,
                                                       const float* b_hh, float* gates_ws, int batch, int c_in, int frames, int ld,
                                                       int hidden, const nbasr_deferred_ln* ln, int batch_total, int batch_offset,
                                                       nbasr_stream_t stream)
{
    clear_error();
    NBASR_REQUIRE(batch_offset >= 0 && batch >= 0 && batch_offset + batch <= batch_total, NBASR_EINVAL,
                  "nbasr_lstm_input_projection_packed_into: utterances %d .. %d do not lie inside a gate tensor of %d", batch_offset,
                  batch_offset + batch, batch_total);
    return pw_projection<PwF16x2>("nbasr_lstm_input_projection_packed", x, ws, packed_w_ih, b_ih, b_hh, gates_ws, batch, c_in, frames, ld, hidden,
                                  ln, batch_total, batch_offset, stream);
}

extern "C" int nbasr_lstm_input_projection_bf16(const void* x, void* ws, const void* packed_w_ih, const float* b_ih, const float* b_hh,
                                                float* gates_ws, int batch, int c_in, int frames, int ld, int hidden,
                                                const nbasr_deferred_ln* ln, nbasr_stream_t stream)
{
    clear_error();
    return pw_projection<PwBf16>("nbasr_lstm_input_projection_bf16", static_cast<const bf16_t*>(x), ws, packed_w_ih, b_ih, b_hh, gates_ws, batch,
                                 c_in, frames, ld, hidden, ln, batch, 0, stream);
}
```

Measured before the change: 11160.

## Make conv and pointwise GEMM kernels persistent with cross-tile operand prefetch

Converts the split-precision conv and pointwise GEMM kernels into persistent kernels that walk tiles with a grid stride. The grid is sized to CUs times resident workgroups, and can be overridden through an environment variable. While the epilogue runs, the first operand slot of the next tile is DMA-prefetched into LDS, and the staging area moves so the two do not overlap. Per-row bias and inverse-scale constants are staged into LDS via async loads instead of being read from global memory in the epilogue. This is meant to hide tile start-up latency and launch tail effects, at the cost of more LDS, more complex barriers and a risk of lower occupancy or load imbalance.

```diff
diff --git a/nb_asr_amd/csrc/gemm_conv_split.hip b/nb_asr_amd/csrc/gemm_conv_split.hip
--- a/nb_asr_amd/csrc/gemm_conv_split.hip
+++ b/nb_asr_amd/csrc/gemm_conv_split.hip
@@ -1,3 +1,4 @@
+#include "persistent_grid.h"
 #include "storage.h"
 
 #include <cstdlib>
@@ -88,6 +89,16 @@
     static constexpr int OPERAND_BYTES = RING * (A_STEP_BYTES + X_BYTES);
     static constexpr int STAGING_BYTES = 8 * 32 * 68 * 4;
     static constexpr int LDS_BYTES = OPERAND_BYTES > STAGING_BYTES ? OPERAND_BYTES : STAGING_BYTES;
+    static constexpr int SLOT_BYTES = A_STEP_BYTES + X_BYTES;
+    static constexpr int CU_LDS_BYTES = 160 * 1024;
+    static constexpr int PREFETCH_LDS_BYTES = OPERAND_BYTES > SLOT_BYTES + STAGING_BYTES ? OPERAND_BYTES : SLOT_BYTES + STAGING_BYTES;
+    static constexpr bool PREFETCH = P::SCALED && X_BYTES % 1024 == 0 && PREFETCH_LDS_BYTES <= CU_LDS_BYTES &&
+                                     CU_LDS_BYTES / PREFETCH_LDS_BYTES == CU_LDS_BYTES / LDS_BYTES;
+    static constexpr int ROWCONST_ROWS = (PBM + 63) / 64 * 64;
+    static constexpr int ROWCONST_BYTES = 2 * ROWCONST_ROWS * 4;
+    static constexpr bool ROWCONST = P::NS > 1;
+    static constexpr int operand_end(bool ximg) { return ximg && PREFETCH ? PREFETCH_LDS_BYTES : LDS_BYTES; }
+    static constexpr int lds_bytes(bool ximg) { return operand_end(ximg) + (ximg && ROWCONST ? 2 * ROWCONST_BYTES : 0); }
     __device__ static constexpr int rowmap(int row) { return (S == 1) ? row : (row & 1) * XRH + (row >> 1); }
 };
 
@@ -97,6 +108,7 @@
     float* y;
     int c_in, frames_in, ld_in, c_out, frames_out, ld_out, lpad;
     int n_groups, n_mt, n_nt, batch;
+    int n_tiles;
     LnRef ln_x;
     const float* x_absmax;
     const float* w_inv_scale;
@@ -187,21 +199,48 @@
     using vec8 = typename P::vec8;
     constexpr int TP = G::TP, QS = G::QSTEPS, ASTEP = G::A_STEP_BYTES;
     extern __shared__ __attribute__((aligned(16))) unsigned char smem[];
+    constexpr int SLOT = G::SLOT_BYTES;
     unsigned char* const Abuf = smem;
-    unsigned char* const Xbase = smem + G::RING * ASTEP;
-
-    const int nwg = gridDim.x, id = blockIdx.x;
-    const int xq = nwg >> 3, xr = nwg & 7, xcd = id & 7;
-    const int L = (xcd < xr ? xcd * (xq + 1) : xr * (xq + 1) + (xcd - xr) * xq) + (id >> 3);
-    int mt_i, b, nt_i;
-    {
-        mt_i = L % a.n_mt;
+    unsigned char* const Xbase = smem + ASTEP;
+    constexpr bool PREFETCH = XIMG && G::PREFETCH;
+    constexpr int STAGE_OFF = PREFETCH ? SLOT : 0;
+    constexpr bool ROWCONST = XIMG && G::ROWCONST;
+    constexpr int RC_OFF = G::operand_end(XIMG);
+    static_assert(!PREFETCH || (STAGE_OFF >= ASTEP + G::X_BYTES && STAGE_OFF + G::STAGING_BYTES <= G::operand_end(XIMG) && G::RING == 2),
+                  "the epilogue's staging and the next tile's first operands must not overlap");
+
+    typedef const __attribute__((address_space(4))) PackedConvArgs* late_args_t;
+    auto late_args = [&]() {
+        if constexpr (XIMG) {
+            late_args_t p = (late_args_t)__builtin_amdgcn_kernarg_segment_ptr();
+            asm volatile("" : "+s"(p));
+            return p;
+        } else {
+            return &a;
+        }
+    };
+    struct Tile { int mt, b, nt; };
+    const unsigned ntiles = a.n_tiles, walk = gridDim.x;
+    auto tile_of = [&](unsigned id) {
+        const auto& a = *late_args();
+        const int xq = ntiles >> 3, xr = ntiles & 7;
+        const int xcd = id & 7;
+        const int L = (xcd < xr ? xcd * (xq + 1) : xr * (xq + 1) + (xcd - xr) * xq) + (id >> 3);
+        Tile t;
+        t.mt = L % a.n_mt;
         const int rest = L / a.n_mt;
-        b = rest / a.n_nt;
-        nt_i = rest - b * a.n_nt;
-    }
-    const int m0 = mt_i * PB_M, n0 = nt_i * PB_N;
-    if (a.x_range && a.sel_want >= 0 && static_cast<int>(range_is_extreme(a.x_range + 4 * b)) != a.sel_want) return;
+        t.b = rest / a.n_nt;
+        t.nt = rest - t.b * a.n_nt;
+        return t;
+    };
+    auto next_id = [&](unsigned id) {
+        const auto& a = *late_args();
+        if (a.x_range && a.sel_want >= 0)
+            while (id < ntiles && static_cast<int>(range_is_extreme(a.x_range + 4 * tile_of(id).b)) != a.sel_want) id += walk;
+        return id;
+    };
+    unsigned id = next_id(blockIdx.x);
+    if (id >= ntiles) return;
 
     const int tid = threadIdx.x;
     const int lane = tid & 63;
@@ -209,20 +248,27 @@
     const int wm = wave >> 2, wn = wave & 3;
     const bool older = wave < 4;
 
-    const float* __restrict__ xb = a.x + static_cast<size_t>(b) * a.c_in * a.ld_in;
-    const int tin0 = n0 * S - a.lpad;
-    const float* __restrict__ xstats = LNX ? a.ln_x.stats + static_cast<size_t>(b) * 2 * a.ld_in : nullptr;
-    const unsigned char* __restrict__ wtile = a.wp + static_cast<size_t>(mt_i) * a.n_groups * pb_group_bytes<P>(MI);
-
-    const bool wave_active = (m0 + wm * WROWS) < a.c_out && (n0 + wn * WCOLS) < a.ld_out;
+    int b, m0, n0, tin0;
+    const float* __restrict__ xb;
+    const float* __restrict__ xstats;
+    const unsigned char* __restrict__ wtile;
+    bool wave_active;
+    int a0, xoff;
+    float x_scale = 1.f, x_inv = 1.f;
+    auto weights_of = [&](const Tile& t) { return a.wp + static_cast<size_t>(t.mt) * a.n_groups * pb_group_bytes<P>(MI); };
+    auto enter_tile = [&](const Tile& t) {
+        const auto& a = *late_args();
+        b = t.b; m0 = t.mt * PB_M; n0 = t.nt * PB_N;
+        tin0 = n0 * S - a.lpad;
+        xb = a.x + static_cast<size_t>(b) * a.c_in * a.ld_in;
+        xstats = LNX ? a.ln_x.stats + static_cast<size_t>(b) * 2 * a.ld_in : nullptr;
+        wtile = weights_of(t);
+        wave_active = (m0 + wm * WROWS) < a.c_out && (n0 + wn * WCOLS) < a.ld_out;
+        a0 = tin0 & ~3; xoff = tin0 - a0;
+        if constexpr (P::SCALED) pow2_normaliser(a.x_range ? a.x_range[4 * b] : a.x_absmax[b], 14, x_scale, x_inv);
+    };
 
     floatx4 acc[MI][NJ], tot[MI][NJ];
-#pragma unroll
-    for (int i = 0; i < MI; ++i)
-#pragma unroll
-        for (int j = 0; j < NJ; ++j)
-#pragma unroll
-            for (int r = 0; r < 4; ++r) { acc[i][j][r] = 0.f; tot[i][j][r] = 0.f; }
     auto flush_group = [&]() {
         if constexpr (P::NS > 1) {
 #pragma unroll
@@ -234,38 +280,68 @@
         }
     };
 
-    auto dma_weights = [&](int step, int buf) {
-        const unsigned char* src = wtile + static_cast<size_t>(step) * ASTEP;
+    auto dma_weights_of = [&](const unsigned char* wt, int step, int buf, int wv) {
+        const unsigned char* src = wt + static_cast<size_t>(step) * ASTEP;
 #pragma unroll
         for (int j = 0; j < ASTEP / 1024 / 8; ++j) {
-            const int chunk = wave * (ASTEP / 1024 / 8) + j;
+            const int chunk = wv * (ASTEP / 1024 / 8) + j;
             __builtin_amdgcn_global_load_lds(
                 (const __attribute__((address_space(1))) void*)(src + chunk * 1024 + lane * 16),
-                (__attribute__((address_space(3))) void*)(Abuf + buf * ASTEP + chunk * 1024),
+                (__attribute__((address_space(3))) void*)(Abuf + buf * SLOT + chunk * 1024),
                 16, 0, 0);
         }
     };
+    auto dma_weights = [&](int step, int buf) { dma_weights_of(wtile, step, buf, wave); };
+    constexpr int NP = (G::X_BYTES + 1023) / 1024;
+    auto image_of = [&](int bb, int g) {
+        return reinterpret_cast<const unsigned char*>(a.x) +
+               (static_cast<size_t>(bb) * a.n_groups + g) * (2 * P::NS) * static_cast<size_t>(a.ld_in + 1) * 16;
+    };
+    auto dma_x_piece = [&](const unsigned char* img, int tin, int xbuf, int i) {
+        const int o = i * 1024 + lane * 16;
+        if (G::X_BYTES % 1024 == 0 || o < G::X_BYTES) {
+            const int plane = o / (G::RP * 16), rr = (o - plane * (G::RP * 16)) >> 4;
+            const int frame = tin + (S == 1 ? rr : 2 * (rr % G::XRH) + rr / G::XRH);
+            const int row = (rr < G::ROWS && frame >= 0 && frame < a.ld_in) ? frame + 1 : 0;
+            __builtin_amdgcn_global_load_lds(
+                (const __attribute__((address_space(1))) void*)(img + (static_cast<size_t>(plane) * (a.ld_in + 1) + row) * 16),
+                (__attribute__((address_space(3))) void*)(Xbase + xbuf * SLOT + i * 1024), 16, 0, 0);
+        }
+    };
     auto dma_x = [&](int g, int xbuf, int q) {
-        constexpr int NP = (G::X_BYTES + 1023) / 1024;
-        const unsigned char* img = reinterpret_cast<const unsigned char*>(a.x) +
-                                   (static_cast<size_t>(b) * a.n_groups + g) * (2 * P::NS) * static_cast<size_t>(a.ld_in + 1) * 16;
+        const unsigned char* img = image_of(b, g);
 #pragma unroll 1
-        for (int i = wave * QS + q; i < NP; i += 8 * QS) {
-            const int o = i * 1024 + lane * 16;
-            if (o < G::X_BYTES) {
-                const int plane = o / (G::RP * 16), rr = (o - plane * (G::RP * 16)) >> 4;
-                const int frame = tin0 + (S == 1 ? rr : 2 * (rr % G::XRH) + rr / G::XRH);
-                const int row = (rr < G::ROWS && frame >= 0 && frame < a.ld_in) ? frame + 1 : 0;
+        for (int i = wave * QS + q; i < NP; i += 8 * QS) dma_x_piece(img, tin0, xbuf, i);
+    };
+    auto dma_row_constants = [&](const Tile& t, int par) {
+        if constexpr (ROWCONST) {
+            const auto& a = *late_args();
+            constexpr int NPC = G::ROWCONST_ROWS / 64;
+            static_assert(2 * NPC <= 8, "one piece per wave");
+            int wv = wave;
+            asm volatile("" : "+s"(wv));
+            if (wv < 2 * NPC) {
+                const bool inv = wv >= NPC;
+                const int row = (inv ? wv - NPC : wv) * 64 + lane;
+                const int m = t.mt * PB_M + (row < PB_M ? row : PB_M - 1);
+                const float* src = inv ? a.w_inv_scale + m : a.bias + min(m, a.c_out - 1);
                 __builtin_amdgcn_global_load_lds(
-                    (const __attribute__((address_space(1))) void*)(img + (static_cast<size_t>(plane) * (a.ld_in + 1) + row) * 16),
-                    (__attribute__((address_space(3))) void*)(Xbase + xbuf * G::X_BYTES + i * 1024), 16, 0, 0);
-            }
-        }
+                    (const __attribute__((address_space(1))) void*)src,
+                    (__attribute__((address_space(3))) void*)(smem + RC_OFF + par * G::ROWCONST_BYTES + wv * 256), 4, 0, 0);
+            }
+        }
+    };
+    auto dma_first_operands = [&](const Tile& t) {
+        int wv = wave;
+        asm volatile("" : "+s"(wv));
+        dma_weights_of(weights_of(t), 0, 0, wv);
+        const unsigned char* img = image_of(t.b, 0);
+        const int tin = t.nt * PB_N * S - a.lpad;
+#pragma unroll
+        for (int k = 0; k < (NP + 7) / 8; ++k)
+            if (wv + 8 * k < NP) dma_x_piece(img, tin, 0, wv + 8 * k);
     };
     floatx4 xreg[G::XI][2];
-    const int a0 = tin0 & ~3, xoff = tin0 - a0;
-    float x_scale = 1.f, x_inv = 1.f;
-    if constexpr (P::SCALED) pow2_normaliser(a.x_range ? a.x_range[4 * b] : a.x_absmax[b], 14, x_scale, x_inv);
     auto load_x = [&](int g, int c) {
 #pragma unroll
         for (int i = 0; i < G::XI; ++i) {
@@ -297,7 +373,7 @@
         }
     };
     auto commit_x = [&](int xbuf, int c) {
-        unsigned* const X = reinterpret_cast<unsigned*>(Xbase + xbuf * G::X_BYTES);
+        unsigned* const X = reinterpret_cast<unsigned*>(Xbase + xbuf * SLOT);
 #pragma unroll
         for (int i = 0; i < G::XI; ++i) {
             const int e = tid + PB_THREADS * (c * G::XI + i);
@@ -325,8 +401,8 @@
 
     constexpr bool PIPE = P::NS <= 2;
     auto mma_step = [&](int q, int abuf, int xbuf) {
-        const unsigned char* A = Abuf + abuf * ASTEP + a_lane;
-        const unsigned char* X = Xbase + xbuf * G::X_BYTES + x_lane;
+        const unsigned char* A = Abuf + abuf * SLOT + a_lane;
+        const unsigned char* X = Xbase + xbuf * SLOT + x_lane;
         auto read_b = [&](int pp, int j, vec8 (&f)[P::NS]) {
             const int row = G::rowmap((wn * WCOLS + j * 16 + l15) * S + q * TP + 2 * pp + (kq >> 1));
 #pragma unroll
@@ -388,17 +464,177 @@
         }
     };
 
+    auto epilogue = [&, tid](int par) {
+    const auto& a = *late_args();
+    int lane_e = tid & 63, wave_e = wave;
+    if constexpr (XIMG) asm volatile("" : "+v"(lane_e), "+s"(wave_e));
+    const int lane = lane_e, l15 = lane & 15, kq = lane >> 4, wm = wave_e >> 2, wn = wave_e & 3;
+    if constexpr (P::NS == 1) {
+        constexpr int TSH = WCOLS + 8;
+        constexpr int LPR = WCOLS / 8, RPI = 64 / LPR;
+        unsigned short* const T = reinterpret_cast<unsigned short*>(smem) + wave_e * (32 * TSH);
+        static_assert(8 * 32 * TSH * 2 <= G::LDS_BYTES, "output staging must fit the operand buffers");
+        if (wave_active) {
+            bf16_t* const yb = reinterpret_cast<bf16_t*>(a.y);
+            const int n = n0 + wn * WCOLS + (lane % LPR) * 8;
+#pragma unroll
+            for (int i0 = 0; i0 < MI; i0 += 2) {
+#pragma unroll
+                for (int ii = 0; ii < 2; ++ii) {
+                    const int i = i0 + ii;
+                    if (i >= MI) break;
+#pragma unroll
+                    for (int j = 0; j < NJ; ++j) {
+                        const bool live = n0 + wn * WCOLS + j * 16 + l15 < a.frames_out;
+#pragma unroll
+                        for (int r = 0; r < 4; ++r) {
+                            const int m = m0 + wm * WROWS + i * 16 + kq * 4 + r;
+                            const float v = (live && m < a.c_out) ? relu_clamp(acc[i][j][r] + a.bias[m]) : 0.f;
+                            T[(ii * 16 + kq * 4 + r) * TSH + j * 16 + l15] = __builtin_bit_cast(unsigned short, static_cast<__bf16>(v));
+                        }
+                    }
+                }
+                asm volatile("s_waitcnt lgkmcnt(0)" ::: "memory");
+                const int rows_pass = (MI - i0 >= 2) ? 32 : 16;
+#pragma unroll
+                for (int it = 0; it < 32 / RPI; ++it) {
+                    const int ml = it * RPI + lane / LPR, m = m0 + wm * WROWS + i0 * 16 + ml;
+                    if (ml < rows_pass && m < a.c_out && n < a.ld_out) {
+                        const u4v t = *reinterpret_cast<const u4v*>(T + ml * TSH + (lane % LPR) * 8);
+                        *reinterpret_cast<u4v*>(yb + (static_cast<size_t>(b) * a.c_out + m) * a.ld_out + n) = t;
+                    }
+                }
+                asm volatile("s_waitcnt lgkmcnt(0)" ::: "memory");
+            }
+        }
+        return;
+    } else {
+    if (XIMG || (!a.s0 && !a.s1 && !a.s2 && a.staged_epilogue)) {
+        constexpr int TS = WCOLS + 4;
+        constexpr int FQ = WCOLS / 4, RI = 64 / FQ, NIT = 32 / RI;
+        float* const T = reinterpret_cast<float*>(smem + STAGE_OFF) + wave_e * (32 * TS);
+        const float* const rc = reinterpret_cast<const float*>(smem + RC_OFF + par * G::ROWCONST_BYTES);
+        static_assert(8 * 32 * TS * 4 <= G::STAGING_BYTES && STAGE_OFF + G::STAGING_BYTES <= G::lds_bytes(XIMG), "output staging must fit the operand buffers");
+        if (!wave_active) return;
+        const int nc = n0 + wn * WCOLS + (lane % FQ) * 4;
+        const bool want_stats = a.part != nullptr;
+        const int scol = lane % WCOLS, usel = lane / WCOLS;
+        const int ncol = n0 + wn * WCOLS + scol;
+#pragma unroll
+        for (int i0 = 0; i0 < MI; i0 += 2) {
+#pragma unroll
+            for (int ii = 0; ii < 2; ++ii) {
+                const int i = i0 + ii;
+                if (i >= MI) break;
+                floatx4 rc_bias, rc_inv;
+                if constexpr (ROWCONST) {
+                    rc_bias = *reinterpret_cast<const floatx4*>(rc + wm * WROWS + i * 16 + kq * 4);
+                    rc_inv = *reinterpret_cast<const floatx4*>(rc + G::ROWCONST_ROWS + wm * WROWS + i * 16 + kq * 4);
+                }
+#pragma unroll
+                for (int j = 0; j < NJ; ++j) {
+                    const bool live = n0 + wn * WCOLS + j * 16 + l15 < a.frames_out;
+#pragma unroll
+                    for (int r = 0; r < 4; ++r) {
+                        const int m = m0 + wm * WROWS + i * 16 + kq * 4 + r;
+                        float v = 0.f;
+                        if (live && m < a.c_out) {
+                            float sum = tot[i][j][r];
+                            if constexpr (P::SCALED) sum = sum * x_inv * (ROWCONST ? rc_inv[r] : a.w_inv_scale[m]);
+                            v = relu_clamp(sum + (ROWCONST ? rc_bias[r] : a.bias[m]));
+                        }
+                        T[(ii * 16 + kq * 4 + r) * TS + j * 16 + l15] = v;
+                    }
+                }
+            }
+            asm volatile("s_waitcnt lgkmcnt(0)" ::: "memory");
+            const int rows_pass = (MI - i0 >= 2) ? 32 : 16;
+#pragma unroll
+            for (int it = 0; it < NIT; ++it) {
+                const int ml = it * RI + lane / FQ;
+                const int m = m0 + wm * WROWS + i0 * 16 + ml;
+                if (ml < rows_pass && m < a.c_out && nc < a.ld_out) {
+                    const floatx4 t = *reinterpret_cast<const floatx4*>(T + ml * TS + (lane % FQ) * 4);
+                    *reinterpret_cast<floatx4*>(a.y + (static_cast<size_t>(b) * a.c_out + m) * a.ld_out + nc) = t;
+                }
+            }
+            if (want_stats) {
+#pragma unroll
+                for (int u0 = 0; u0 < 2; u0 += 64 / WCOLS) {
+                    const int u = u0 + usel;
+                    const int mu = m0 + wm * WROWS + (i0 + u) * 16;
+                    if (i0 + u < MI && mu < a.c_out) {
+                        const int nrows = min(16, a.c_out - mu);
+                        const float c = T[(u * 16) * TS + scol];
+                        float s1 = 0.f, s2 = 0.f;
+#pragma unroll
+                        for (int r = 1; r < 16; ++r) {
+                            const float d = (r < nrows) ? T[(u * 16 + r) * TS + scol] - c : 0.f;
+                            s1 += d;
+                            s2 = __builtin_fmaf(d, d, s2);
+                        }
+                        if (ncol < a.ld_out) {
+                            const float inv = 1.0f / static_cast<float>(nrows);
+                            float* prow = a.part + (static_cast<size_t>(mu >> 4) * a.batch + b) * 2 * a.ld_out + ncol;
+                            prow[0] = c + s1 * inv;
+                            prow[a.ld_out] = s2 - s1 * s1 * inv;
+                        }
+                    }
+                }
+            }
+            asm volatile("s_waitcnt lgkmcnt(0)" ::: "memory");
+        }
+        return;
+    }
+    if (!wave_active) return;
+#pragma unroll
+    for (int i = 0; i < MI; ++i) {
+#pragma unroll
+        for (int j = 0; j < NJ; ++j) {
+            const int n = n0 + wn * WCOLS + j * 16 + l15;
+            if (n >= a.ld_out) continue;
+            const bool live = n < a.frames_out;
+#pragma unroll
+            for (int r = 0; r < 4; ++r) {
+                const int m = m0 + wm * WROWS + i * 16 + kq * 4 + r;
+                if (m >= a.c_out) continue;
+                float sum = tot[i][j][r];
+                if constexpr (P::SCALED) sum = sum * x_inv * a.w_inv_scale[m];
+                float v = relu_clamp(sum + a.bias[m]);
+                const size_t off = (static_cast<size_t>(b) * a.c_out + m) * a.ld_out + n;
+                if (a.s0) v += a.s0[off];
+                if (a.s1) v += a.s1[off];
+                if (a.s2) v += a.s2[off];
+                a.y[off] = live ? v : 0.f;
+            }
+        }
+    }
+    }
+    };
+
     const int ng = a.n_groups;
-    dma_weights(0, 0);
-    if constexpr (XIMG) {
+    int par = 0;
+    for (bool first = true;; first = false) {
+    enter_tile(tile_of(id));
+    if (first || !PREFETCH) {
+        dma_row_constants(tile_of(id), par);
+        dma_weights(0, 0);
+        if constexpr (XIMG) {
 #pragma unroll 1
-        for (int q = 0; q < QS; ++q) dma_x(0, 0, q);
-    } else {
+            for (int q = 0; q < QS; ++q) dma_x(0, 0, q);
+        } else {
 #pragma unroll 1
-        for (int c = 0; c < G::NCHUNK; ++c) { load_x(0, c); commit_x(0, c); }
+            for (int c = 0; c < G::NCHUNK; ++c) { load_x(0, c); commit_x(0, c); }
+        }
     }
     asm volatile("s_waitcnt vmcnt(0)" ::: "memory");
     __syncthreads();
+#pragma unroll
+    for (int i = 0; i < MI; ++i)
+#pragma unroll
+        for (int j = 0; j < NJ; ++j)
+#pragma unroll
+            for (int r = 0; r < 4; ++r) { acc[i][j][r] = 0.f; tot[i][j][r] = 0.f; }
 
     if (!older) __builtin_amdgcn_s_setprio(1);
     int step = 0;
@@ -433,141 +669,20 @@
         }
         flush_group();
     }
-
-    if constexpr (P::NS == 1) {
-        constexpr int TSH = WCOLS + 8;
-        constexpr int LPR = WCOLS / 8, RPI = 64 / LPR;
-        unsigned short* const T = reinterpret_cast<unsigned short*>(smem) + wave * (32 * TSH);
-        static_assert(8 * 32 * TSH * 2 <= G::LDS_BYTES, "output staging must fit the operand buffers");
-        if (wave_active) {
-            bf16_t* const yb = reinterpret_cast<bf16_t*>(a.y);
-            const int n = n0 + wn * WCOLS + (lane % LPR) * 8;
-#pragma unroll
-            for (int i0 = 0; i0 < MI; i0 += 2) {
-#pragma unroll
-                for (int ii = 0; ii < 2; ++ii) {
-                    const int i = i0 + ii;
-                    if (i >= MI) break;
-#pragma unroll
-                    for (int j = 0; j < NJ; ++j) {
-                        const bool live = n0 + wn * WCOLS + j * 16 + l15 < a.frames_out;
-#pragma unroll
-                        for (int r = 0; r < 4; ++r) {
-                            const int m = m0 + wm * WROWS + i * 16 + kq * 4 + r;
-                            const float v = (live && m < a.c_out) ? relu_clamp(acc[i][j][r] + a.bias[m]) : 0.f;
-                            T[(ii * 16 + kq * 4 + r) * TSH + j * 16 + l15] = __builtin_bit_cast(unsigned short, static_cast<__bf16>(v));
-                        }
-                    }
-                }
-                asm volatile("s_waitcnt lgkmcnt(0)" ::: "memory");
-                const int rows_pass = (MI - i0 >= 2) ? 32 : 16;
-#pragma unroll
-                for (int it = 0; it < 32 / RPI; ++it) {
-                    const int ml = it * RPI + lane / LPR, m = m0 + wm * WROWS + i0 * 16 + ml;
-                    if (ml < rows_pass && m < a.c_out && n < a.ld_out) {
-                        const u4v t = *reinterpret_cast<const u4v*>(T + ml * TSH + (lane % LPR) * 8);
-                        *reinterpret_cast<u4v*>(yb + (static_cast<size_t>(b) * a.c_out + m) * a.ld_out + n) = t;
-                    }
-                }
-                asm volatile("s_waitcnt lgkmcnt(0)" ::: "memory");
-            }
-        }
-        return;
-    } else {
-    if (!a.s0 && !a.s1 && !a.s2 && a.staged_epilogue) {
-        constexpr int TS = WCOLS + 4;
-        constexpr int FQ = WCOLS / 4, RI = 64 / FQ, NIT = 32 / RI;
-        float* const T = reinterpret_cast<float*>(smem) + wave * (32 * TS);
-        static_assert(8 * 32 * TS * 4 <= G::LDS_BYTES, "output staging must fit the operand buffers");
-        if (!wave_active) return;
-        const int nc = n0 + wn * WCOLS + (lane % FQ) * 4;
-        const bool want_stats = a.part != nullptr;
-        const int scol = lane % WCOLS, usel = lane / WCOLS;
-        const int ncol = n0 + wn * WCOLS + scol;
-#pragma unroll
-        for (int i0 = 0; i0 < MI; i0 += 2) {
-#pragma unroll
-            for (int ii = 0; ii < 2; ++ii) {
-                const int i = i0 + ii;
-                if (i >= MI) break;
-#pragma unroll
-                for (int j = 0; j < NJ; ++j) {
-                    const bool live = n0 + wn * WCOLS + j * 16 + l15 < a.frames_out;
-#pragma unroll
-                    for (int r = 0; r < 4; ++r) {
-                        const int m = m0 + wm * WROWS + i * 16 + kq * 4 + r;
-                        float v = 0.f;
-                        if (live && m < a.c_out) {
-                            float sum = tot[i][j][r];
-                            if constexpr (P::SCALED) sum = sum * x_inv * a.w_inv_scale[m];
-                            v = relu_clamp(sum + a.bias[m]);
-                        }
-                        T[(ii * 16 + kq * 4 + r) * TS + j * 16 + l15] = v;
-                    }
-                }
-            }
-            asm volatile("s_waitcnt lgkmcnt(0)" ::: "memory");
-            const int rows_pass = (MI - i0 >= 2) ? 32 : 16;
-#pragma unroll
-            for (int it = 0; it < NIT; ++it) {
-                const int ml = it * RI + lane / FQ;
-                const int m = m0 + wm * WROWS + i0 * 16 + ml;
-                if (ml < rows_pass && m < a.c_out && nc < a.ld_out) {
-                    const floatx4 t = *reinterpret_cast<const floatx4*>(T + ml * TS + (lane % FQ) * 4);
-                    *reinterpret_cast<floatx4*>(a.y + (static_cast<size_t>(b) * a.c_out + m) * a.ld_out + nc) = t;
-                }
-            }
-            if (want_stats) {
-#pragma unroll
-                for (int u0 = 0; u0 < 2; u0 += 64 / WCOLS) {
-                    const int u = u0 + usel;
-                    const int mu = m0 + wm * WROWS + (i0 + u) * 16;
-                    if (i0 + u < MI && mu < a.c_out) {
-                        const int nrows = min(16, a.c_out - mu);
-                        const float c = T[(u * 16) * TS + scol];
-                        float s1 = 0.f, s2 = 0.f;
-#pragma unroll
-                        for (int r = 1; r < 16; ++r) {
-                            const float d = (r < nrows) ? T[(u * 16 + r) * TS + scol] - c : 0.f;
-                            s1 += d;
-                            s2 = __builtin_fmaf(d, d, s2);
-                        }
-                        if (ncol < a.ld_out) {
-                            const float inv = 1.0f / static_cast<float>(nrows);
-                            float* prow = a.part + (static_cast<size_t>(mu >> 4) * a.batch + b) * 2 * a.ld_out + ncol;
-                            prow[0] = c + s1 * inv;
-                            prow[a.ld_out] = s2 - s1 * s1 * inv;
-                        }
-                    }
-                }
-            }
-            asm volatile("s_waitcnt lgkmcnt(0)" ::: "memory");
-        }
-        return;
-    }
-    if (!wave_active) return;
-#pragma unroll
-    for (int i = 0; i < MI; ++i) {
-#pragma unroll
-        for (int j = 0; j < NJ; ++j) {
-            const int n = n0 + wn * WCOLS + j * 16 + l15;
-            if (n >= a.ld_out) continue;
-            const bool live = n < a.frames_out;
-#pragma unroll
-            for (int r = 0; r < 4; ++r) {
-                const int m = m0 + wm * WROWS + i * 16 + kq * 4 + r;
-                if (m >= a.c_out) continue;
-                float sum = tot[i][j][r];
-                if constexpr (P::SCALED) sum = sum * x_inv * a.w_inv_scale[m];
-                float v = relu_clamp(sum + a.bias[m]);
-                const size_t off = (static_cast<size_t>(b) * a.c_out + m) * a.ld_out + n;
-                if (a.s0) v += a.s0[off];
-                if (a.s1) v += a.s1[off];
-                if (a.s2) v += a.s2[off];
-                a.y[off] = live ? v : 0.f;
-            }
-        }
-    }
+    if (XIMG && !older) __builtin_amdgcn_s_setprio(0);
+
+    const unsigned next = next_id(id + walk);
+    if constexpr (PREFETCH) {
+        if (next < ntiles) {
+            dma_first_operands(tile_of(next));
+            dma_row_constants(tile_of(next), par ^ 1);
+        }
+    }
+    epilogue(par);
+    if (!XIMG || next >= ntiles) return;
+    if constexpr (!PREFETCH) __syncthreads();
+    id = next;
+    par ^= 1;
     }
 }
 
@@ -590,12 +705,13 @@
     NBASR_REQUIRE(HAS_LNX || !a.ln_x.stats, NBASR_EINVAL, "%s: this scheme takes no deferred LayerNorm", P::NAME);
     a.n_mt = (a.c_out + PB_M - 1) / PB_M;
     a.n_nt = (a.ld_out + G::PBN - 1) / G::PBN;
-    const long long nwg = static_cast<long long>(a.n_mt) * a.n_nt * a.batch;
-    NBASR_REQUIRE(nwg < (1ll << 31), NBASR_EINVAL, "%s: too many tiles (%lld)", P::NAME, nwg);
+    const long long tiles = static_cast<long long>(a.n_mt) * a.n_nt * a.batch;
+    NBASR_REQUIRE(tiles < (1ll << 31), NBASR_EINVAL, "%s: too many tiles (%lld)", P::NAME, tiles);
+    a.n_tiles = static_cast<int>(tiles);
     if (a.ln_x.stats)
-        hipLaunchKernelGGL((gemm_conv_split_kernel<P, S, HAS_LNX>), dim3(static_cast<unsigned>(nwg)), dim3(PB_THREADS), G::LDS_BYTES, stream, a);
+        hipLaunchKernelGGL((gemm_conv_split_kernel<P, S, HAS_LNX>), dim3(static_cast<unsigned>(tiles)), dim3(PB_THREADS), G::LDS_BYTES, stream, a);
     else
-        hipLaunchKernelGGL((gemm_conv_split_kernel<P, S, false>), dim3(static_cast<unsigned>(nwg)), dim3(PB_THREADS), G::LDS_BYTES, stream, a);
+        hipLaunchKernelGGL((gemm_conv_split_kernel<P, S, false>), dim3(static_cast<unsigned>(tiles)), dim3(PB_THREADS), G::LDS_BYTES, stream, a);
     return launch_status(P::NAME);
 }
 
@@ -605,17 +721,21 @@
 static int launch_image(PackedConvArgs a, hipStream_t stream)
 {
     using G = GeoP<P, S, MI, NJ>;
-    static const hipError_t attr = hipFuncSetAttribute(reinterpret_cast<const void*>(gemm_conv_split_kernel<P, S, false, true, MI, NJ>),
-                                                       hipFuncAttributeMaxDynamicSharedMemorySize, G::LDS_BYTES);
+    constexpr int LDS = G::lds_bytes(true);
+    const void* const kernel = reinterpret_cast<const void*>(gemm_conv_split_kernel<P, S, false, true, MI, NJ>);
+    static const hipError_t attr = hipFuncSetAttribute(kernel, hipFuncAttributeMaxDynamicSharedMemorySize, LDS);
     if (attr != hipSuccess) {
-        set_error("%s: cannot reserve %d bytes of LDS: %s", P::NAME, G::LDS_BYTES, hipGetErrorString(attr));
+        set_error("%s: cannot reserve %d bytes of LDS: %s", P::NAME, LDS, hipGetErrorString(attr));
         return static_cast<int>(attr);
     }
+    static const int per_cu = resident_workgroups_per_cu(kernel, PB_THREADS, LDS);
+    constexpr bool WALK = S == 1;
     a.n_mt = (a.c_out + G::PBM - 1) / G::PBM;
     a.n_nt = (a.ld_out + G::PBN - 1) / G::PBN;
-    const long long nwg = static_cast<long long>(a.n_mt) * a.n_nt * a.batch;
-    NBASR_REQUIRE(nwg < (1ll << 31), NBASR_EINVAL, "%s: too many tiles (%lld)", P::NAME, nwg);
-    hipLaunchKernelGGL((gemm_conv_split_kernel<P, S, false, true, MI, NJ>), dim3(static_cast<unsigned>(nwg)), dim3(PB_THREADS), G::LDS_BYTES, stream, a);
+    const long long tiles = static_cast<long long>(a.n_mt) * a.n_nt * a.batch;
+    NBASR_REQUIRE(tiles < (1ll << 31), NBASR_EINVAL, "%s: too many tiles (%lld)", P::NAME, tiles);
+    a.n_tiles = static_cast<int>(tiles);
+    hipLaunchKernelGGL((gemm_conv_split_kernel<P, S, false, true, MI, NJ>), dim3(persistent_grid(per_cu, tiles, WALK)), dim3(PB_THREADS), LDS, stream, a);
     return launch_status(P::NAME);
 }
 
diff --git a/nb_asr_amd/csrc/gemm_pointwise.hip b/nb_asr_amd/csrc/gemm_pointwise.hip
--- a/nb_asr_amd/csrc/gemm_pointwise.hip
+++ b/nb_asr_amd/csrc/gemm_pointwise.hip
@@ -1,3 +1,4 @@
+#include "persistent_grid.h"
 #include "storage.h"
 
 namespace nbasr {
@@ -19,7 +20,12 @@
     static constexpr int A_STEP = TERMS * 2 * 2 * PW_M * 16;
     static constexpr int X_STEP = TERMS * 2 * 2 * PW_N * 16;
     static constexpr int RING = 3;
-    static constexpr int LDS = RING * (A_STEP + X_STEP);
+    static constexpr int SLOT = A_STEP + X_STEP;
+    static constexpr int LDS = RING * SLOT;
+    static constexpr int STAGING = 8 * 16 * 68 * 4;
+    template <bool SWAP> static constexpr bool prefetch() { return SWAP && RING == 3 && SLOT >= STAGING; }
+    static constexpr int ROWCONST_BYTES = 3 * 128 * 4 + 256;
+    template <bool SWAP> static constexpr int lds_bytes() { return LDS + (SWAP ? 2 * ROWCONST_BYTES : 0); }
     static constexpr int DMA_PER_WAVE = 3 * TERMS;
 };
 
@@ -197,6 +203,7 @@
     const typename P::act_t* s0; const typename P::act_t* s1; const typename P::act_t* s2;
     void* y;
     int c_out, frames, ld_out, n_ks, n_mt, n_nt, batch;
+    int n_tiles;
     int n_major;
     int row_stride_t, row_stride_b;
     LnRef ln_s0;
@@ -209,58 +216,99 @@
     typedef typename P::act_t act_t;
     constexpr int NS = P::NS, A_STEP = P::A_STEP, X_STEP = P::X_STEP;
     extern __shared__ __attribute__((aligned(16))) unsigned char smem[];
+    constexpr int SLOT = P::SLOT;
     unsigned char* const Abuf = smem;
-    unsigned char* const Xbuf = smem + P::RING * A_STEP;
-
-    const int nwg = gridDim.x, id = blockIdx.x;
-    const int xq = nwg >> 3, xr = nwg & 7, xcd = id & 7;
-    const int L = (xcd < xr ? xcd * (xq + 1) : xr * (xq + 1) + (xcd - xr) * xq) + (id >> 3);
-    int mt_i, b, nt_i;
-    if (!P::ORDER_BY_HOST || a.n_major) {
-        const int ntg = L / a.n_mt;
-        mt_i = L - ntg * a.n_mt;
-        b = ntg / a.n_nt;
-        nt_i = ntg - b * a.n_nt;
-    } else {
-        const int per_m = a.n_nt * a.batch;
-        mt_i = L / per_m;
-        const int rem = L - mt_i * per_m;
-        b = rem / a.n_nt;
-        nt_i = rem - b * a.n_nt;
-    }
-    const int m0 = mt_i * PW_M, n0 = nt_i * PW_N;
+    unsigned char* const Xbuf = smem + A_STEP;
+    constexpr bool WALK = SWAP, PREFETCH = P::template prefetch<SWAP>(), ROWCONST = SWAP;
+    constexpr int STAGE_OFF = PREFETCH ? 2 * SLOT : 0, RC_OFF = P::LDS;
+    static_assert(!PREFETCH || STAGE_OFF + P::STAGING <= P::LDS, "the epilogue's staging and the next tile's first K-steps must not overlap");
+
+    typedef const __attribute__((address_space(4))) PointwiseArgs<P>* late_args_t;
+    auto late_args = [&]() {
+        if constexpr (WALK) {
+            late_args_t p = (late_args_t)__builtin_amdgcn_kernarg_segment_ptr();
+            asm volatile("" : "+s"(p));
+            return p;
+        } else {
+            return &a;
+        }
+    };
+    struct Tile { int mt, b, nt; };
+    const unsigned ntiles = a.n_tiles, walk = gridDim.x;
+    auto tile_of = [&](unsigned id) {
+        const auto& a = *late_args();
+        const int xq = a.n_tiles >> 3, xr = a.n_tiles & 7, xcd = id & 7;
+        const int L = (xcd < xr ? xcd * (xq + 1) : xr * (xq + 1) + (xcd - xr) * xq) + (id >> 3);
+        Tile t;
+        if (!P::ORDER_BY_HOST || a.n_major) {
+            const int ntg = L / a.n_mt;
+            t.mt = L - ntg * a.n_mt;
+            t.b = ntg / a.n_nt;
+            t.nt = ntg - t.b * a.n_nt;
+        } else {
+            const int per_m = a.n_nt * a.batch;
+            t.mt = L / per_m;
+            const int rem = L - t.mt * per_m;
+            t.b = rem / a.n_nt;
+            t.nt = rem - t.b * a.n_nt;
+        }
+        return t;
+    };
+    unsigned id = blockIdx.x;
 
     const int tid = threadIdx.x, lane = tid & 63;
     const int wave = __builtin_amdgcn_readfirstlane(tid >> 6);
     const int wm = wave >> 2, wn = wave & 3;
     const int l15 = lane & 15, kq = lane >> 4;
-    const bool wave_active = (m0 + wm * 64) < a.c_out && (n0 + wn * 64) < a.ld_out;
-
-    const unsigned char* __restrict__ wsrc = a.wp + static_cast<size_t>(mt_i) * a.n_ks * A_STEP;
-    const unsigned char* __restrict__ xsrc = a.image + (static_cast<size_t>(b) * a.n_nt + nt_i) * a.n_ks * X_STEP;
+
+    int b, nt_i, m0, n0;
+    bool wave_active;
+    const unsigned char* __restrict__ wsrc;
+    const unsigned char* __restrict__ xsrc;
+    auto weights_of = [&](const Tile& t) { return a.wp + static_cast<size_t>(t.mt) * a.n_ks * A_STEP; };
+    auto image_of = [&](const Tile& t) { return a.image + (static_cast<size_t>(t.b) * a.n_nt + t.nt) * a.n_ks * X_STEP; };
+    auto enter_tile = [&](const Tile& t) {
+        const auto& a = *late_args();
+        b = t.b; nt_i = t.nt; m0 = t.mt * PW_M; n0 = t.nt * PW_N;
+        wave_active = (m0 + wm * 64) < a.c_out && (n0 + wn * 64) < a.ld_out;
+        wsrc = weights_of(t);
+        xsrc = image_of(t);
+    };
 
     floatx4 big[4][4], small[4][4];
-#pragma unroll
-    for (int i = 0; i < 4; ++i)
-#pragma unroll
-        for (int j = 0; j < 4; ++j)
-#pragma unroll
-            for (int r = 0; r < 4; ++r) { big[i][j][r] = 0.f; small[i][j][r] = 0.f; }
-
-    auto dma_step = [&](int ks, int buf) {
+
+    auto dma_step_of = [&](const unsigned char* wsrc, const unsigned char* xsrc, int ks, int buf, int wv) {
         const unsigned char* ws = wsrc + static_cast<size_t>(ks) * A_STEP;
         const unsigned char* xs = xsrc + static_cast<size_t>(ks) * X_STEP;
 #pragma unroll
         for (int j = 0; j < NS; ++j) {
-            const int piece = wave * NS + j;
+            const int piece = wv * NS + j;
             __builtin_amdgcn_global_load_lds((const __attribute__((address_space(1))) void*)(ws + piece * 1024 + lane * 16),
-                                             (__attribute__((address_space(3))) void*)(Abuf + buf * A_STEP + piece * 1024), 16, 0, 0);
+                                             (__attribute__((address_space(3))) void*)(Abuf + buf * SLOT + piece * 1024), 16, 0, 0);
         }
 #pragma unroll
         for (int j = 0; j < 2 * NS; ++j) {
-            const int piece = wave * 2 * NS + j;
+            const int piece = wv * 2 * NS + j;
             __builtin_amdgcn_global_load_lds((const __attribute__((address_space(1))) void*)(xs + piece * 1024 + lane * 16),
-                                             (__attribute__((address_space(3))) void*)(Xbuf + buf * X_STEP + piece * 1024), 16, 0, 0);
+                                             (__attribute__((address_space(3))) void*)(Xbuf + buf * SLOT + piece * 1024), 16, 0, 0);
+        }
+    };
+    auto dma_step = [&](int ks, int buf) { dma_step_of(wsrc, xsrc, ks, buf, wave); };
+    auto dma_row_constants = [&](const Tile& t, int par) {
+        if constexpr (ROWCONST) {
+            const auto& a = *late_args();
+            int wv = wave;
+            asm volatile("" : "+s"(wv));
+            const int arr = wv >> 1;
+            const float* base = arr == 0 ? (P::SCALED ? a.w_inv : nullptr) : (arr == 1 ? a.bias : (arr == 2 ? a.bias2 : nullptr));
+            if (P::SCALED && wv == 6) base = a.x_inv;
+            if (base) {
+                const int m = t.mt * PW_M + (wv & 1) * 64 + lane;
+                const size_t at = wv == 6 ? static_cast<size_t>(t.b) * a.n_nt + t.nt : (arr == 0 ? m : min(m, a.c_out - 1));
+                __builtin_amdgcn_global_load_lds(
+                    (const __attribute__((address_space(1))) void*)(base + at),
+                    (__attribute__((address_space(3))) void*)(smem + RC_OFF + par * P::ROWCONST_BYTES + wv * 256), 4, 0, 0);
+            }
         }
     };
 
@@ -268,8 +316,8 @@
     const int x_lane = ((kq * PW_N) + wn * 64 + l15) * 16;
 
     auto mma_step = [&](int buf) {
-        const unsigned char* A = Abuf + buf * A_STEP + a_lane;
-        const unsigned char* X = Xbuf + buf * X_STEP + x_lane;
+        const unsigned char* A = Abuf + buf * SLOT + a_lane;
+        const unsigned char* X = Xbuf + buf * SLOT + x_lane;
         auto read_a = [&](int i, vec8 (&f)[NS]) {
 #pragma unroll
             for (int s = 0; s < NS; ++s) f[s] = *reinterpret_cast<const vec8*>(A + s * (A_STEP / NS) + i * 16 * 16);
@@ -301,13 +349,25 @@
 
     const bool older = wave < 4;
     const int n_ks = a.n_ks;
-    dma_step(0, 0);
-    if (n_ks > 1) {
-        dma_step(1, 1);
-        asm volatile("s_waitcnt vmcnt(%0)\n\ts_barrier" :: "n"(P::DMA_PER_WAVE) : "memory");
-    } else {
-        asm volatile("s_waitcnt vmcnt(0)\n\ts_barrier" ::: "memory");
-    }
+    int par = 0;
+    for (bool first = true;; first = false) {
+    enter_tile(tile_of(id));
+    const bool two_steps = late_args()->n_ks > 1;
+    if (first || !PREFETCH) {
+        int wv = wave;
+        asm volatile("" : "+s"(wv));
+        dma_row_constants(tile_of(id), par);
+        dma_step_of(wsrc, xsrc, 0, 0, wv);
+        if (two_steps) dma_step_of(wsrc, xsrc, 1, 1, wv);
+    }
+    if (two_steps) asm volatile("s_waitcnt vmcnt(%0)\n\ts_barrier" :: "n"(P::DMA_PER_WAVE) : "memory");
+    else          asm volatile("s_waitcnt vmcnt(0)\n\ts_barrier" ::: "memory");
+#pragma unroll
+    for (int i = 0; i < 4; ++i)
+#pragma unroll
+        for (int j = 0; j < 4; ++j)
+#pragma unroll
+            for (int r = 0; r < 4; ++r) { big[i][j][r] = 0.f; small[i][j][r] = 0.f; }
     if (!older) __builtin_amdgcn_s_setprio(1);
     int buf = 0;
 #pragma unroll 1
@@ -323,19 +383,49 @@
     }
     if (!older) __builtin_amdgcn_s_setprio(0);
 
+    const unsigned next = id + walk;
+    if constexpr (PREFETCH) {
+        if (next < ntiles) {
+            const Tile t = tile_of(next);
+            int wv = wave;
+            asm volatile("" : "+s"(wv));
+            dma_row_constants(t, par ^ 1);
+            dma_step_of(weights_of(t), image_of(t), 0, 0, wv);
+            if (two_steps) dma_step_of(weights_of(t), image_of(t), 1, 1, wv);
+        }
+    }
+
+    [&, tid]() {
+    const auto& a = *late_args();
+    int lane_e = tid & 63, wave_e = wave;
+    if constexpr (WALK) asm volatile("" : "+v"(lane_e), "+s"(wave_e));
+    const int lane = lane_e, l15 = lane & 15, kq = lane >> 4, wave = wave_e, wm = wave >> 2, wn = wave & 3;
+    (void)lane;
     if (!wave_active) return;
+    const float* const rc = reinterpret_cast<const float*>(smem + RC_OFF + par * P::ROWCONST_BYTES);
     float x_inv = 1.f;
-    if constexpr (P::SCALED) x_inv = a.x_inv[static_cast<size_t>(b) * a.n_nt + nt_i];
+    if constexpr (P::SCALED) x_inv = ROWCONST ? rc[3 * PW_M] : a.x_inv[static_cast<size_t>(b) * a.n_nt + nt_i];
+    const bool has_bias2 = a.bias2 != nullptr;
+    floatx4 rc_inv[4], rc_bias[4], rc_bias2[4];
+    if constexpr (ROWCONST) {
+#pragma unroll
+        for (int i = 0; i < 4; ++i) {
+            const float* row = rc + wm * 64 + i * 16 + kq * 4;
+            if constexpr (P::SCALED) rc_inv[i] = *reinterpret_cast<const floatx4*>(row);
+            rc_bias[i] = *reinterpret_cast<const floatx4*>(row + PW_M);
+            rc_bias2[i] = *reinterpret_cast<const floatx4*>(row + 2 * PW_M);
+        }
+    }
     auto product = [&](int i, int j, int r, int m) {
         float v = big[i][j][r];
         if constexpr (NS == 2) v += small[i][j][r] * (1.f / 2048.f);
-        if constexpr (P::SCALED) v = v * x_inv * a.w_inv[m];
+        if constexpr (P::SCALED) v = v * x_inv * (ROWCONST ? rc_inv[i][r] : a.w_inv[m]);
         return v;
     };
     if constexpr (SWAP) {
         constexpr int TS = 64 + 4;
-        static_assert(8 * 16 * TS * 4 <= P::LDS, "output staging must fit the operand buffers");
-        float* const T = reinterpret_cast<float*>(smem) + wave * (16 * TS);
+        static_assert(8 * 16 * TS * 4 == P::STAGING && STAGE_OFF + P::STAGING <= P::LDS, "output staging must fit the operand buffers");
+        float* const T = reinterpret_cast<float*>(smem + STAGE_OFF) + wave * (16 * TS);
         const int mseg = m0 + wm * 64 + l15 * 4;
 #pragma unroll
         for (int j = 0; j < 4; ++j) {
@@ -348,8 +438,8 @@
                     const int m = mb + r;
                     float v = 0.f;
                     if (m < a.c_out) {
-                        v = product(i, j, r, m) + a.bias[m];
-                        if (a.bias2) v += a.bias2[m];
+                        v = product(i, j, r, m) + (ROWCONST ? rc_bias[i][r] : a.bias[m]);
+                        if (has_bias2) v += (ROWCONST ? rc_bias2[i][r] : a.bias2[m]);
                         if (RELU) v = relu_clamp(v);
                     }
                     o[r] = v;
@@ -398,6 +488,13 @@
             }
         }
     }
+    }();
+
+    if (!WALK || next >= ntiles) return;
+    if constexpr (!PREFETCH) asm volatile("s_waitcnt lgkmcnt(0)\n\ts_barrier" ::: "memory");
+    id = next;
+    par ^= 1;
+    }
 }
 
 static inline int pw_n_ks(int c_in) { return (c_in + PW_K - 1) / PW_K; }
@@ -484,16 +581,20 @@
     }
     a.c_out = c_out; a.frames = frames; a.ld_out = ld; a.batch = batch;
 
-    static const hipError_t attr = hipFuncSetAttribute(reinterpret_cast<const void*>(pw_gemm_kernel<P, SWAP, RELU>),
-                                                       hipFuncAttributeMaxDynamicSharedMemorySize, P::LDS);
+    constexpr int LDS = P::template lds_bytes<SWAP>();
+    const void* const kernel = reinterpret_cast<const void*>(pw_gemm_kernel<P, SWAP, RELU>);
+    static const hipError_t attr = hipFuncSetAttribute(kernel, hipFuncAttributeMaxDynamicSharedMemorySize, LDS);
     if (attr != hipSuccess) {
-        set_error("%s: cannot reserve %d bytes of LDS: %s", what, P::LDS, hipGetErrorString(attr));
+        set_error("%s: cannot reserve %d bytes of LDS: %s", what, LDS, hipGetErrorString(attr));
         return static_cast<int>(attr);
     }
-    const long long nwg = static_cast<long long>(a.n_mt) * a.n_nt * a.batch;
-    NBASR_REQUIRE(nwg < (1ll << 31), NBASR_EINVAL, "%s: too many tiles (%lld)", what, nwg);
+    static const int per_cu = SWAP ? resident_workgroups_per_cu(kernel, PW_THREADS, LDS) : 0;
+    const long long tiles = static_cast<long long>(a.n_mt) * a.n_nt * a.batch;
+    NBASR_REQUIRE(tiles < (1ll << 31), NBASR_EINVAL, "%s: too many tiles (%lld)", what, tiles);
+    a.n_tiles = static_cast<int>(tiles);
+    const unsigned grid = SWAP ? persistent_grid(per_cu, tiles) : static_cast<unsigned>(tiles);
     a.n_major = static_cast<long long>(a.n_mt) * P::A_STEP <= static_cast<long long>(a.n_nt) * a.batch * P::X_STEP ? 1 : 0;
-    hipLaunchKernelGGL((pw_gemm_kernel<P, SWAP, RELU>), dim3(static_cast<unsigned>(nwg)), dim3(PW_THREADS), P::LDS, stream, a);
+    hipLaunchKernelGGL((pw_gemm_kernel<P, SWAP, RELU>), dim3(grid), dim3(PW_THREADS), LDS, stream, a);
     return launch_status(what);
 }
 
diff --git a/nb_asr_amd/csrc/persistent_grid.h b/nb_asr_amd/csrc/persistent_grid.h
--- /dev/null
+++ b/nb_asr_amd/csrc/persistent_grid.h
@@ -0,0 +1,42 @@
+#pragma once
+#include "common.h"
+
+#include <cstdlib>
+
+namespace nbasr {
+
+inline int device_compute_units()
+{
+    static const int n = [] {
+        int dev = 0;
+        hipDeviceProp_t prop;
+        if (hipGetDevice(&dev) != hipSuccess || hipGetDeviceProperties(&prop, dev) != hipSuccess) return 0;
+        return prop.multiProcessorCount;
+    }();
+    return n;
+}
+
+inline int resident_workgroups_per_cu(const void* kernel, int threads, size_t lds)
+{
+    int n = 0;
+    if (hipOccupancyMaxActiveBlocksPerMultiprocessor(&n, kernel, threads, lds) != hipSuccess) {
+        (void)hipGetLastError();
+        return 0;
+    }
+    return n;
+}
+
+inline unsigned persistent_grid(int per_cu, long long tiles, bool walk = true)
+{
+    long long g = walk ? static_cast<long long>(device_compute_units()) * per_cu : 0;
+    g -= g % 8;
+    if (g <= 0 || g > tiles) g = tiles;
+    if (const char* env = std::getenv("NBASR_GEMM_GRID")) {
+        char* end = nullptr;
+        const long long n = std::strtoll(env, &end, 10);
+        if (end != env) g = n < 1 ? 1 : (n > tiles ? tiles : n);
+    }
+    return static_cast<unsigned>(g);
+}
+
+}
```

After: 11220, median of 6. No clear change (+0.6%).
